# ZZWaang/polyphonic-chord-texture-disentanglement

Measured on AMD Instinct MI355X. Metric: 2-bar piano-roll samples/sec (train step), higher is better.
Workload: dtype bf16; 1 GPU; configs[1]: 1xMI355X batch=512/GPU, bf16 MFMA GRU/Linear, z_dim=256+256, teacher-forced decoder (tfr=1), fwd+bwd+clip+Adam; per_gpu_batch=512, global_batch=512, parallelism=dp1

## Files before the change

include/ptvae_hip.h:

```cpp
#ifndef PTVAE_HIP_H
#define PTVAE_HIP_H

#ifdef __cplusplus
extern "C" {
#endif

#define PTV_PREC_F32 0
#define PTV_PREC_BF16 1

#define PTV_A_BF16 1
#define PTV_B_BF16 2
#define PTV_C_BF16 4
#define PTV_GRU_GATES_BF16 1
#define PTV_GRU_GI_BF16 2
#define PTV_GRU_GI2_BF16 4
#define PTV_GRU_DG_BF16 8
#define PTV_GRU_W_BF16 16
#define PTV_GRU_EXT_BF16 64
#define PTV_GRU_SKIP_CAST0 32

const char* ptv_arch(void);
int ptv_abi_version(void);
const char* ptv_header_hash(void);

int ptv_gemm(int prec, int transA, int transB, int M, int N, int K,
             const void* A, long lda, const void* B, long ldb,
             void* C, long ldc, const float* bias, float alpha,
             int accumulate, int act, int splitk, int dtypes, void* stream);
int ptv_gemm_mtop(int prec, int transA, int transB, int M, int N, int K, const void* A, long lda, const void* B, long ldb,
                  void* C, long ldc, const float* bias, float alpha, int accumulate, int act, int splitk, int dtypes,
                  const int* m_top, long m_unit, void* stream);
int ptv_gemm_mtop_seg(int prec, int transA, int transB, int M, int N, int K, const void* A, long lda, const void* B, long ldb,
                      void* C, long ldc, const float* bias, float alpha, int accumulate, int act, int splitk, int dtypes,
                      const int* m_top, long m_unit, const int* seg_n, long seg_unit, int seg_period, void* stream);
int ptv_gemm_priority(int p);

int ptv_gru_seq_fwd(int prec, int M, int H, int T,
                    const void* gi, long gi_step_stride, long gi_ld,
                    const void* gi2, long gi2_step_stride, long gi2_ld,
                    const void* w_hh, const float* b_hh,
                    float* hall, void* hall16, void* gates,
                    const int* lengths, int reverse, const int* gi_idx, int flags, void* stream);

int ptv_gru_step_fwd(int prec, int M, int H,
                     const float* hprev, long ld_hprev, const void* hprev16, void* hout16,
                     const void* gi, long gi_ld, const void* gi2, long gi2_ld,
                     const void* w_hh, const float* b_hh,
                     float* hout, long ld_hout,
                     void* gates, long gates_plane,
                     const int* lengths, int t, const int* gi_idx, int flags, void* stream);

int ptv_gru_seq_bwd(int prec, int M, int H, int T,
                    const float* hall, const void* gates, const void* w_hh,
                    const void* dh_ext, long ext_step_stride, long ext_ld,
                    const float* dh_last, long last_ld,
                    const float* lr_a, long lr_step_stride, long lr_lda, int lr_k, const float* lr_b,
                    void* dgi, void* dgh, float* dhz, float* dh0,
                    int reverse, int flags, void* stream);

int ptv_gru_persist_supported(int NC, int M, int H);
int ptv_gru_persist_cu_reserve(int cus);
int ptv_gru_persist_load_policy(int lp);
int ptv_gru_persist_fwd(int NC, int M, int H, int T,
                        const void* const* gi, const long* gi_step, const long* gi_ld,
                        const void* const* gi2, const long* gi2_step, const long* gi2_ld,
                        const void* const* w_hh16, const float* const* b_hh,
                        float* const* hall, void* const* hall16, void* const* gates,
                        const int* const* lengths, const int* reverse, void* const* xch, unsigned* sync, void* stream);
int ptv_gru_persist_bwd(int NC, int M, int H, int T,
                        const float* const* hall, const void* const* gates, const void* const* w_t16,
                        const void* const* dh_ext, const long* ext_step, const long* ext_ld, const int* ext_bf16,
                        const float* const* dh_last, const long* last_ld,
                        void* const* dgi, void* const* dgh, float* const* dh0,
                        const int* reverse, void* const* xch, unsigned* sync, void* stream);
int ptv_gru_persist_splitk_supported(int NC, int M, int H, int S);
long ptv_gru_persist_part_elems(int NC, int M, int H, int S);
int ptv_gru_persist_bwd_splitk(int S, int NC, int M, int H, int T,
                               const float* const* hall, const void* const* gates, const void* const* w_t16,
                               const void* const* dh_ext, const long* ext_step, const long* ext_ld, const int* ext_bf16,
                               const float* const* dh_last, const long* last_ld,
                               void* const* dgi, void* const* dgh, float* const* dh0,
                               const int* reverse, void* const* xch, float* const* part, unsigned* sync, void* stream);

int ptv_copy2d(float* dst, long ldd, const float* src, long lds, long rows, int cols, float alpha,
               int accumulate, void* stream);
int ptv_transpose01(float* dst, const float* src, int D0, int D1, int W, void* stream);
int ptv_sum_steps(float* out, const void* in, long n, int T, long stride, int accumulate, int in_bf16, void* stream);
int ptv_zero_skip(int enable);
int ptv_last_nonzero_unit(const float* x, long rows, int cols, long ld, long unit, int* top, void* stream);
int ptv_sum_steps_top(float* out, const void* in, long n, int T, long stride, int accumulate, int in_bf16, const int* t_top,
                      void* stream);
int ptv_sum_steps_seg(float* out, const void* in, long n, int T, long stride, int accumulate, int in_bf16, const int* t_top,
                      const int* seg_n, long row_elems, void* stream);
int ptv_colsum(float* out, const void* A, long lda, long rows, int N, const int* sel, int G, int a_bf16, void* stream);

int ptv_embed_fwd(const long* x, const float* W, const float* bias, float* emb, int* lengths, int B, int E, void* stream);
int ptv_multihot(const long* x, float* out, long ld, int B, void* stream);
int ptv_grid_lengths(const long* x, int* lengths, int B, void* stream);
int ptv_multihot_bf16(const long* x, void* out, long ld, int B, void* stream);
int ptv_embed_fwd_geom(const long* x, const float* W, const float* bias, float* emb, int* lengths, int B, int E,
                       int S, int N, int P, int D, int pad, void* stream);
int ptv_grid_lengths_geom(const long* x, int* lengths, int B, int S, int N, int D, int pad, void* stream);
int ptv_multihot_geom(const long* x, void* out, long ld, int B, int S, int N, int P, int D, int bf16, void* stream);
int ptv_embed_multihot_fwd(const unsigned char* mh, const float* W, const float* bias, float* emb, int* lengths,
                           int B, int E, int S, int N, int K, int pad_col, void* stream);
int ptv_multihot_bytes_rows(const unsigned char* mh, void* out, long ld, int B, int S, int N, int K, int bf16, void* stream);

int ptv_txt_conv_relu_pool_fwd(const float* pr_mat, const float* w, const float* bias, float* pooled, int B, int C, void* stream);
int ptv_txt_conv_relu_pool_bwd(const float* pr_mat, const float* w, const float* bias, const float* dpooled,
                               float* dw, float* dbias, int B, int C, void* stream);
int ptv_txt_conv_relu_pool_fwd_rows(const float* pr_mat, const float* w, const float* bias, float* feat, long ld, int B, int C,
                                    signed char* arg, void* stream);
int ptv_txt_conv_relu_pool_bwd_rows(const float* pr_mat, const float* w, const float* bias, const float* dfeat, long ld,
                                    float* dw, float* dbias, int B, int C, const signed char* arg, void* stream);

int ptv_philox_normal(float* out, long rows, int Z, unsigned long long seed, unsigned long long stream_id, long row_offset,
                      void* stream);
// ... 119 lines not shown

enum PtvCdfTensor {
  PTV_CDF_Z = 0,
  PTV_CDF_C_SM,
  PTV_CDF_W_ZHID, PTV_CDF_B_ZHID, PTV_CDF_W_ZIN, PTV_CDF_B_ZIN, PTV_CDF_INIT_INPUT,
  PTV_CDF_W_IH,
  PTV_CDF_B_IH, PTV_CDF_W_HH, PTV_CDF_B_HH, PTV_CDF_W_ROOT, PTV_CDF_B_ROOT, PTV_CDF_W_CHROMA, PTV_CDF_B_CHROMA, PTV_CDF_W_BASS, PTV_CDF_B_BASS,
  PTV_CDF_HALL,
  PTV_CDF_Z_IN,
  PTV_CDF_TOKS,
  PTV_CDF_GI,
  PTV_CDF_ZG,
  PTV_CDF_GATES,
  PTV_CDF_ROOT, PTV_CDF_CHROMA, PTV_CDF_BASS,
  PTV_CDF_COUNT
};
enum PtvCdfDim { PTV_CDF_D_B = 0, PTV_CDF_D_T, PTV_CDF_D_H, PTV_CDF_D_I, PTV_CDF_D_Z, PTV_CDF_D_ZI, PTV_CDF_D_PREC, PTV_CDF_D_GATES_BF16,
                 PTV_CDF_D_NROOT, PTV_CDF_D_NCHROMA, PTV_CDF_D_NBASS, PTV_CDF_D_COUNT };
int ptv_chord_decoder_fwd(const void* const* t, const long* d, void* stream);

enum PtvCdbTensor {
  PTV_CDB_Z = 0,
  PTV_CDB_W_ZHID, PTV_CDB_W_ZIN, PTV_CDB_W_IH, PTV_CDB_W_HH, PTV_CDB_W_ROOT, PTV_CDB_W_CHROMA, PTV_CDB_W_BASS,
  PTV_CDB_WT16_HH,
  PTV_CDB_HALL, PTV_CDB_GATES, PTV_CDB_TOKS, PTV_CDB_Z_IN,
  PTV_CDB_DROOT, PTV_CDB_DCHROMA, PTV_CDB_DBASS,
  PTV_CDB_DZ,
  PTV_CDB_G_INIT_INPUT, PTV_CDB_G_W_ZHID, PTV_CDB_G_B_ZHID, PTV_CDB_G_W_ZIN, PTV_CDB_G_B_ZIN, PTV_CDB_G_W_IH, PTV_CDB_G_B_IH, PTV_CDB_G_W_HH,
  PTV_CDB_G_B_HH, PTV_CDB_G_W_ROOT, PTV_CDB_G_B_ROOT, PTV_CDB_G_W_CHROMA, PTV_CDB_G_B_CHROMA, PTV_CDB_G_W_BASS, PTV_CDB_G_B_BASS,
  PTV_CDB_DHS,
  PTV_CDB_DGI, PTV_CDB_DGH,
  PTV_CDB_DHZ,
  PTV_CDB_DH0,
  PTV_CDB_DZG,
  PTV_CDB_DZ_IN,
  PTV_CDB_DTOK0,
  PTV_CDB_XCH, PTV_CDB_PART, PTV_CDB_SYNC,
  PTV_CDB_WAIT_EVENT, PTV_CDB_RECORD_EVENT,
  PTV_CDB_COUNT
};
enum PtvCdbDim { PTV_CDB_D_B = 0, PTV_CDB_D_T, PTV_CDB_D_H, PTV_CDB_D_I, PTV_CDB_D_Z, PTV_CDB_D_ZI, PTV_CDB_D_PREC, PTV_CDB_D_ACT_BF16,
                 PTV_CDB_D_NROOT, PTV_CDB_D_NCHROMA, PTV_CDB_D_NBASS, PTV_CDB_D_PERSIST, PTV_CDB_D_SPLITK, PTV_CDB_D_COUNT };
int ptv_chord_decoder_bwd(const void* const* tensors, const long* dims, void* stream);

enum PtvDtbTensor {
  PTV_DTB_Z = 0,
  PTV_DTB_TOK_OP,
  PTV_DTB_DP,
  PTV_DTB_DDUR,
  PTV_DTB_TOP_H,
  PTV_DTB_W_HH_D, PTV_DTB_B_HH_D, PTV_DTB_W_IH_D, PTV_DTB_W_OUT_D, PTV_DTB_SOS,
  PTV_DTB_PK_WDPT, PTV_DTB_PK_WCAT,
  PTV_DTB_PK_NOTES_WT,
  PTV_DTB_WT_IH_N, PTV_DTB_WT_T2N, PTV_DTB_WT_IH_T, PTV_DTB_WT_HH_T, PTV_DTB_WT_ZHID, PTV_DTB_WT_ZIN,
  PTV_DTB_NS, PTV_DTB_NS16, PTV_DTB_Z_IN, PTV_DTB_TOKS, PTV_DTB_GATES_T, PTV_DTB_HN16, PTV_DTB_GATES_N, PTV_DTB_PITCH, PTV_DTB_HD16,
  PTV_DTB_TAB0, PTV_DTB_TAB, PTV_DTB_IDX,
  PTV_DTB_DZ,
  PTV_DTB_DTOK,
  PTV_DTB_DTOKS,
  PTV_DTB_G_W_ZHID, PTV_DTB_G_B_ZHID, PTV_DTB_G_W_ZIN, PTV_DTB_G_B_ZIN, PTV_DTB_G_INIT_INPUT,
  PTV_DTB_G_W_IH_T, PTV_DTB_G_W_HH_T, PTV_DTB_G_B_IH_T, PTV_DTB_G_B_HH_T,
  PTV_DTB_G_W_T2N, PTV_DTB_G_B_T2N,
  PTV_DTB_G_W_IH_N, PTV_DTB_G_W_HH_N, PTV_DTB_G_B_IH_N, PTV_DTB_G_B_HH_N,
  PTV_DTB_G_W_P, PTV_DTB_G_B_P, PTV_DTB_G_W_DH, PTV_DTB_G_B_DH, PTV_DTB_G_W_OUT_D, PTV_DTB_G_B_OUT_D,
  PTV_DTB_G_W_IH_D, PTV_DTB_G_W_HH_D, PTV_DTB_G_B_IH_D, PTV_DTB_G_B_HH_D, PTV_DTB_G_SOS,
  PTV_DTB_DHD0,
  PTV_DTB_PART,
  PTV_DTB_S,
  PTV_DTB_TMP64,
  PTV_DTB_DNSUM,
  PTV_DTB_DY16,
  PTV_DTB_TMP200,
  PTV_DTB_CS200,
  PTV_DTB_DGI_N, PTV_DTB_DGH_N, PTV_DTB_DHN0, PTV_DTB_SCRATCH_N,
  PTV_DTB_TOP_STEP,
  PTV_DTB_DGC, PTV_DTB_DNS,
  PTV_DTB_DGI_T, PTV_DTB_DGH_T, PTV_DTB_DZHID, PTV_DTB_DZG, PTV_DTB_DZ_IN,
  PTV_DTB_XCH, PTV_DTB_PART_T, PTV_DTB_SYNC,
  PTV_DTB_WAIT_EVENT, PTV_DTB_RECORD_EVENT,
  PTV_DTB_SIDE_STREAM,
  PTV_DTB_FORK_EVENT0, PTV_DTB_FORK_EVENT1, PTV_DTB_FORK_EVENT2, PTV_DTB_FORK_EVENT3,
  PTV_DTB_PERM, PTV_DTB_ROW_LEN,
  PTV_DTB_NS16S,
  PTV_DTB_DNS_S,
  PTV_DTB_DTOK_S,
  PTV_DTB_SEG_N,
  PTV_DTB_COUNT
};
enum PtvDtbDim { PTV_DTB_D_B = 0, PTV_DTB_D_E, PTV_DTB_D_HE, PTV_DTB_D_HT, PTV_DTB_D_HN, PTV_DTB_D_HD, PTV_DTB_D_NP, PTV_DTB_D_ZS, PTV_DTB_D_ZI,
                 PTV_DTB_D_LDP, PTV_DTB_D_NBLK, PTV_DTB_D_SPLITK, PTV_DTB_D_COUNT };
int ptv_decoder_tf_bwd(const void* const* tensors, const long* dims, void* stream);

enum PtvBgbTensor {
  PTV_BGB_X = 0,
  PTV_BGB_DOUT,
  PTV_BGB_HALL0, PTV_BGB_H16_0, PTV_BGB_GATES0, PTV_BGB_WT_HH0, PTV_BGB_WT_IH0,
  PTV_BGB_HALL1, PTV_BGB_H16_1, PTV_BGB_GATES1, PTV_BGB_WT_HH1, PTV_BGB_WT_IH1,
  PTV_BGB_G_W_IH0, PTV_BGB_G_W_HH0, PTV_BGB_G_B_IH0, PTV_BGB_G_B_HH0, PTV_BGB_G_W_IH1, PTV_BGB_G_W_HH1, PTV_BGB_G_B_IH1, PTV_BGB_G_B_HH1,
  PTV_BGB_DX,
  PTV_BGB_DGI0, PTV_BGB_DGH0, PTV_BGB_DGI1, PTV_BGB_DGH1,
  PTV_BGB_XCH0, PTV_BGB_XCH1, PTV_BGB_PART0, PTV_BGB_PART1, PTV_BGB_SYNC,
  PTV_BGB_WAIT_EVENT, PTV_BGB_RECORD_EVENT, PTV_BGB_SIDE_STREAM, PTV_BGB_FORK_EVENT, PTV_BGB_JOIN_EVENT,
  PTV_BGB_COUNT
};
enum PtvBgbDim { PTV_BGB_D_M = 0, PTV_BGB_D_T, PTV_BGB_D_H, PTV_BGB_D_I, PTV_BGB_D_X_BF16, PTV_BGB_D_DX_ACC, PTV_BGB_D_SPLITK, PTV_BGB_D_COUNT };
int ptv_bigru_final_bwd(const void* const* tensors, const long* dims, void* stream);

enum PtvBgfTensor {
  PTV_BGF_X = 0,
  PTV_BGF_LENGTHS,
  PTV_BGF_W16_IH0, PTV_BGF_B_IH0, PTV_BGF_W16_HH0, PTV_BGF_B_HH0, PTV_BGF_W16_IH1, PTV_BGF_B_IH1, PTV_BGF_W16_HH1, PTV_BGF_B_HH1,
  PTV_BGF_OUT,
  PTV_BGF_GI0, PTV_BGF_HALL0, PTV_BGF_H16_0, PTV_BGF_GATES0, PTV_BGF_GI1, PTV_BGF_HALL1, PTV_BGF_H16_1, PTV_BGF_GATES1,
  PTV_BGF_XCH0, PTV_BGF_XCH1, PTV_BGF_SYNC, PTV_BGF_WAIT_EVENT, PTV_BGF_RECORD_EVENT,
  PTV_BGF_COUNT
};
enum PtvBgfDim { PTV_BGF_D_M = 0, PTV_BGF_D_T, PTV_BGF_D_H, PTV_BGF_D_I, PTV_BGF_D_X_BF16,
                 PTV_BGF_D_WIH_F32,
                 PTV_BGF_D_COUNT };
int ptv_bigru_final_fwd(const void* const* tensors, const long* dims, void* stream);

enum PtvBrfTensor {
  PTV_BRF_X = 0,
  PTV_BRF_LENGTHS, PTV_BRF_PERM,
  PTV_BRF_PK_WG_H0, PTV_BRF_PK_WG_T0, PTV_BRF_B_HH0, PTV_BRF_B_IH0, PTV_BRF_PK_WG_H1, PTV_BRF_PK_WG_T1, PTV_BRF_B_HH1, PTV_BRF_B_IH1,
  PTV_BRF_OUT,
  PTV_BRF_HALL0, PTV_BRF_H16_0, PTV_BRF_GATES0, PTV_BRF_HALL1, PTV_BRF_H16_1, PTV_BRF_GATES1,
  PTV_BRF_SIDE_STREAM, PTV_BRF_FORK_EVENT, PTV_BRF_JOIN_EVENT,
  PTV_BRF_COUNT
};
enum PtvBrfDim { PTV_BRF_D_M = 0, PTV_BRF_D_T, PTV_BRF_D_H, PTV_BRF_D_I, PTV_BRF_D_COUNT };
int ptv_bigru_rows_fwd(const void* const* tensors, const long* dims, void* stream);
enum PtvBrbTensor {
  PTV_BRB_X = 0, PTV_BRB_DOUT, PTV_BRB_LENGTHS, PTV_BRB_PERM,
  PTV_BRB_PK_WT0, PTV_BRB_HALL0, PTV_BRB_H16_0, PTV_BRB_GATES0, PTV_BRB_WT_IH0,
  PTV_BRB_PK_WT1, PTV_BRB_HALL1, PTV_BRB_H16_1, PTV_BRB_GATES1, PTV_BRB_WT_IH1,
  PTV_BRB_G_W_IH0, PTV_BRB_G_W_HH0, PTV_BRB_G_B_IH0, PTV_BRB_G_B_HH0, PTV_BRB_G_W_IH1, PTV_BRB_G_W_HH1, PTV_BRB_G_B_IH1, PTV_BRB_G_B_HH1,
  PTV_BRB_DX,
  PTV_BRB_DGI0, PTV_BRB_DGH0, PTV_BRB_SCRATCH0, PTV_BRB_TOP0, PTV_BRB_DGI1, PTV_BRB_DGH1, PTV_BRB_SCRATCH1, PTV_BRB_TOP1,
  PTV_BRB_SIDE_STREAM, PTV_BRB_FORK_EVENT, PTV_BRB_JOIN_EVENT,
  PTV_BRB_SEG,
  PTV_BRB_COUNT
};
enum PtvBrbDim { PTV_BRB_D_M = 0, PTV_BRB_D_T, PTV_BRB_D_H, PTV_BRB_D_I, PTV_BRB_D_DX_ACC, PTV_BRB_D_DOUT_LD, PTV_BRB_D_COUNT };
int ptv_bigru_rows_bwd(const void* const* tensors, const long* dims, void* stream);

enum PtvVlTensor {
  PTV_VL_X = 0, PTV_VL_C,
  PTV_VL_PITCH, PTV_VL_DUR,
  PTV_VL_MU_C, PTV_VL_SD_C, PTV_VL_MU_R, PTV_VL_SD_R,
  PTV_VL_ROOT, PTV_VL_CHROMA, PTV_VL_BASS,
  PTV_VL_PITCH_T, PTV_VL_DUR_T, PTV_VL_COUNTS, PTV_VL_ROOT_T, PTV_VL_CHROMA_T, PTV_VL_BASS_T,
  PTV_VL_SUMS,
  PTV_VL_OUT,
  PTV_VL_GOUT,
  PTV_VL_GS,
  PTV_VL_DPITCH, PTV_VL_DDUR, PTV_VL_DMU_C, PTV_VL_DSD_C, PTV_VL_DMU_R, PTV_VL_DSD_R, PTV_VL_DROOT, PTV_VL_DCHROMA, PTV_VL_DBASS,
  PTV_VL_COUNT
};
enum PtvVlDim { PTV_VL_D_B = 0, PTV_VL_D_Z, PTV_VL_D_NP, PTV_VL_D_LDP, PTV_VL_D_SM_P, PTV_VL_D_SM_C, PTV_VL_D_HAVE_TARGETS, PTV_VL_D_COUNT };
int ptv_vae_loss_fwd(const void* const* tensors, const long* dims, const double* scal, void* stream);
int ptv_vae_loss_bwd(const void* const* tensors, const long* dims, const double* scal, void* stream);

int ptv_note_token(const float* pitch, long ld_pitch, const int* dur_idx, long dur_stride, const float* W, const float* bias, int E,
                   float* pred, long ld_pred, long* xhat, long xhat_stride, int* plen, int n, int last,
                   const int* force_pitch, int M, void* stream);
int ptv_chord_token(const float* root, const float* chroma, const float* bass, unsigned* masks2, float* token, int B, void* stream);
int ptv_route_slices(const float* src, float* dstA, float* dstB, const int* mask, long slice_elems, int nslices, int accumulate, void* stream);
// ... 30 lines not shown
int ptv_free_resummarize(const void* const* w, const void* const* io, int B, int t, int train, void* stream);

enum PtvDffTensor {
  PTV_DFF_Z = 0,
  PTV_DFF_XS,
  PTV_DFF_TOK0_SRC,
  PTV_DFF_W_ZHID, PTV_DFF_B_ZHID, PTV_DFF_W_ZIN, PTV_DFF_B_ZIN, PTV_DFF_W_IH_T, PTV_DFF_B_IH_T, PTV_DFF_INIT_INPUT, PTV_DFF_B_HH_T,
  PTV_DFF_W_IH_T_OP,
  PTV_DFF_W_HH_T_OP,
  PTV_DFF_W_CAT, PTV_DFF_B_CAT,
  PTV_DFF_W_IH_N, PTV_DFF_B_IH_N, PTV_DFF_B_HH_N, PTV_DFF_W_DH, PTV_DFF_B_DH, PTV_DFF_W_HH_D, PTV_DFF_B_HH_D, PTV_DFF_TAB0, PTV_DFF_TAB,
  PTV_DFF_W_OUT_D, PTV_DFF_B_OUT_D, PTV_DFF_PK_NOTES_H, PTV_DFF_PK_NOTES_T,
  PTV_DFF_PK_E_H0, PTV_DFF_PK_E_T0, PTV_DFF_B_HH_E0, PTV_DFF_B_IH_E0, PTV_DFF_PK_E_H1, PTV_DFF_PK_E_T1, PTV_DFF_B_HH_E1, PTV_DFF_B_IH_E1,
  PTV_DFF_NS, PTV_DFF_NS16, PTV_DFF_Z_IN, PTV_DFF_ZG, PTV_DFF_TOKS, PTV_DFF_GATES_T,
  PTV_DFF_GI, PTV_DFF_H0GC,
  PTV_DFF_TOK, PTV_DFF_PRED, PTV_DFF_PITCH, PTV_DFF_HN, PTV_DFF_HN16, PTV_DFF_GATES_N, PTV_DFF_HD, PTV_DFF_HD16, PTV_DFF_GATES_D,
  PTV_DFF_IDX, PTV_DFF_PLEN, PTV_DFF_GC16, PTV_DFF_DUR_SCR, PTV_DFF_IDX_SCR,
  PTV_DFF_XH0, PTV_DFF_XH1, PTV_DFF_XH16_0, PTV_DFF_XH16_1, PTV_DFF_XG0, PTV_DFF_XG1,
  PTV_DFF_WAIT_EVENT, PTV_DFF_RECORD_EVENT,
  PTV_DFF_SAMPLE,
  PTV_DFF_COUNT
};
enum PtvDffDim {
  PTV_DFF_D_B = 0, PTV_DFF_D_ZS, PTV_DFF_D_ZI, PTV_DFF_D_HE, PTV_DFF_D_HT, PTV_DFF_D_HN, PTV_DFF_D_HD, PTV_DFF_D_E, PTV_DFF_D_NP,
  PTV_DFF_D_LDP,
  PTV_DFF_D_TRAIN, PTV_DFF_D_REPLAY, PTV_DFF_D_INFERENCE,
  PTV_DFF_D_LOOP_FLAGS,
  PTV_DFF_D_CLUSTER,
  PTV_DFF_D_RESUM_TRAIN,
  PTV_DFF_D_TOK0_LDS,
  PTV_DFF_D_W_IH_T_BF16, PTV_DFF_D_W_HH_T_BF16,
  PTV_DFF_D_COUNT
};
int ptv_decoder_free_fwd(const void* const* t, const long* d, const void* const* wl, const void* const* io, const void* const* wr,
                         const void* const* ior, const unsigned* note_mask, const unsigned char* time_coin, void* stream);

enum PtvDfbTensor {
  PTV_DFB_DTOK = 0,
  PTV_DFB_DTOKS,
  PTV_DFB_DEMB, PTV_DFB_DPRED,
  PTV_DFB_DXS, PTV_DFB_DXSP,
  PTV_DFB_MASK_TOK, PTV_DFB_MASK_TIME,
  PTV_DFB_DX_PRED,
  PTV_DFB_XHAT,
  PTV_DFB_MH,
  PTV_DFB_G_W_EMB, PTV_DFB_G_B_EMB,
  PTV_DFB_COUNT
};
enum PtvDfbDim { PTV_DFB_D_B = 0, PTV_DFB_D_E, PTV_DFB_D_HE, PTV_DFB_D_COUNT };
int ptv_decoder_free_bwd(const void* const* t_tf, const long* d_tf, const void* const* t_rows, const long* d_rows, const void* const* t,
                         const long* d, void* stream);

int ptv_notes_gru_persist_fwd(const void* wg_h, const void* wg_t, const float* b_hh, const void* gc, const float* emb,
                              const float* h0, void* HN16, void* gates, long R, int T, void* stream);
int ptv_notes_gru_persist_fwd_top(const void* wg_h, const void* wg_t, const float* b_hh, const void* gc, const float* emb,
                                  const float* h0, void* HN16, void* gates, long R, int T, const int* live_top, void* stream);
long ptv_notes_gru_persist_scratch_elems(long R);
int ptv_notes_gru_persist_bwd(const void* wt, const void* HN16, const void* gates, const void* ext, void* dgi, void* dgh,
                              float* dh0, void* scratch, long R, int T, int* top_step, void* stream);
int ptv_notes_gru_persist_bwd_top(const void* wt, const void* HN16, const void* gates, const void* ext, void* dgi, void* dgh,
                                  float* dh0, void* scratch, long R, int T, const int* bound, int* top_step, void* stream);
int ptv_notes_gru_persist_fwd_rows(const void* wg_h, const void* wg_t, const float* b_hh, const void* gc, const float* emb,
                                   const float* h0, void* HN16, void* gates, long R, int T, const int* live_top, const int* row_len,
                                   void* stream);
int ptv_notes_gru_persist_bwd_rows(const void* wt, const void* HN16, const void* gates, const void* ext, void* dgi, void* dgh,
                                   float* dh0, void* scratch, long R, int T, const int* bound, const int* row_len, int* top_step,
                                   void* stream);
int ptv_notes_bwd_variant(int eight_waves);

int ptv_row_gru_persist_fwd(int H, const void* w_hh, const void* w_x, const float* b_hh, const float* b_ih, const void* gc,
                            const float* x, long x_step, const int* lengths, float* HN, void* HN16, void* gates,
                            float* out, long out_ld, long R, int T, int reverse, void* stream);
long ptv_row_gru_persist_scratch_elems(int H, long R);
int ptv_row_gru_persist_bwd(int H, const void* wt, const void* HN, const void* gates, const void* ext,
                            const float* dh_last, long last_ld, const int* lengths, void* dgi, void* dgh, float* dh0,
                            void* scratch, long R, int T, int reverse, int* top_step, void* stream);
int ptv_row_gru_persist_fwd_perm(int H, const void* w_hh, const void* w_x, const float* b_hh, const float* b_ih, const void* gc,
                                 const float* x, long x_step, const int* lengths, const int* perm, float* HN, void* HN16,
                                 void* gates, float* out, long out_ld, long R, int T, int reverse, void* stream);
int ptv_row_gru_persist_bwd_perm(int H, const void* wt, const void* HN, const void* gates, const void* ext,
                                 const float* dh_last, long last_ld, const int* lengths, const int* perm, void* dgi, void* dgh,
                                 float* dh0, void* scratch, long R, int T, int reverse, int* top_step, void* stream);
int ptv_rows_by_length(const int* lengths, int* perm, long R, int max_len, void* stream);

int ptv_cast_bf16(const float* src, void* dst, long n, void* stream);
int ptv_transpose_cast_bf16(const float* src, void* dst, int rows, int cols, void* stream);
int ptv_transpose_cast_bf16_batched(const float* flat, void* flat_t, const long* desc, int nmat, long ntiles, void* stream);
int ptv_grad_sumsq(const float* g, long n, float* sumsq, void* stream);
int ptv_clip_adam_step(float* p, const float* g, float* m, float* v, long n, const float* sumsq, float gscale, float clip,
                       float lr, float beta1, float beta2, float eps, int step, void* stream);
int ptv_clip_adam_step_shadow(float* p, const float* g, float* m, float* v, long n, const float* sumsq, float gscale, float clip,
                              float lr, float beta1, float beta2, float eps, int step, void* p16, void* stream);
int ptv_gradnorm_clip_adam_step(float* p, const float* g, float* m, float* v, long n, float* sumsq, float gscale, float clip,
                                float lr, float beta1, float beta2, float eps, int step, void* p16, void* stream);

int ptv_ordered_reductions(int on);
int ptv_wgrad_mode(int ordered);
int ptv_wgrad_dma(int enable);
long ptv_ordered_fallbacks(int reset);

int ptv_step_params(const float* dev4);

int ptv_wgrad(int M, int N, int K, const void* A, long lda, const void* B, long ldb, float* C, long ldc, float alpha,
              int accumulate, int dtypes, int slabs, float* colsum_a, const int* k_top, long k_unit, int k_rev, void* stream);
int ptv_wgrad_cat(int M1, const void* A1, long lda1, int M2, const void* A2, long lda2, int N, int K, const void* B, long ldb,
                  float* C, long ldc, float alpha, int accumulate, int dtypes, int slabs, float* colsum_a, const int* k_top,
                  long k_unit, int k_rev, void* stream);
typedef struct ptv_wgrad_job {
  int M, N, K;
  const void* A; long lda;
  const void* B; long ldb;
  float* C; long ldc;
  float alpha;
  int accumulate, dtypes, slabs;
  float* colsum_a;
  const int* k_top; long k_unit; int k_rev;
  const int* seg_n; long seg_unit; int seg_period;
} ptv_wgrad_job;
int ptv_wgrad_batch(const ptv_wgrad_job* jobs, int njobs, void* stream);
int ptv_wgrad_seg_supported(long K, long seg_unit);
int ptv_rows_seg_counts(const int* row_len, long R, int steps, int* seg_n, void* stream);


#ifdef __cplusplus
}
#endif
#endif
```

polyphonic_chord_texture_disentanglement_amd/csrc/composite.hip:

```cpp
#include "common.hpp"
#include "../../include/ptvae_hip.h"

namespace {

inline const void* T_(const void* const* t, int i) { return t[i]; }
template <typename X> inline X* M_(const void* const* t, int i) { return reinterpret_cast<X*>(const_cast<void*>(t[i])); }

constexpr int A16 = 1, B16 = 2, C16 = 4, CBLK16 = 16;

struct WgradGroup {
  ptv_wgrad_job jobs[8]; int n = 0; int P; void* stream;
  WgradGroup(int prec, void* st) : P(prec), stream(st) {}
  int add(int M, int N, long K, const void* A, long lda, int a_bf16, const void* B, long ldb, int b_bf16, float* C, long ldc, float* csum,
          const int* k_top = nullptr, long k_unit = 0, int k_rev = 0, int accumulate = 1, const int* seg_n = nullptr, long seg_unit = 0,
          int seg_period = 0) {
    if (P == PTV_PREC_BF16 && K >= 512) {
      if (n == 8) PTV_TRY(flush());
      jobs[n++] = ptv_wgrad_job{M, N, (int)K, A, lda, B, ldb, C, ldc, 1.f, accumulate, (a_bf16 ? 1 : 0) | (b_bf16 ? 2 : 0), 0, csum, k_top, k_unit, k_rev,
                                seg_n, seg_n ? seg_unit : 0, seg_n ? seg_period : 0};
      return PTV_OK;
    }
    if (k_top) return PTV_ERR_ARG;
    PTV_TRY(ptv_gemm(P, 1, 1, M, N, (int)K, A, lda, B, ldb, C, ldc, nullptr, 1.f, accumulate, 0, 0, (a_bf16 ? A16 : 0) | (b_bf16 ? B16 : 0), stream));
    if (csum) PTV_TRY(ptv_colsum(csum, A, lda, K, M, nullptr, 1, a_bf16, stream));
// ... 128 lines not shown
                   0, 0, 0, stream));
  return PTV_OK;
}

extern "C" int ptv_chord_decoder_bwd(const void* const* t, const long* d, void* stream) {
  if (!t || !d) return PTV_ERR_ARG;
  const int B = (int)d[PTV_CDB_D_B], T = (int)d[PTV_CDB_D_T], H = (int)d[PTV_CDB_D_H], I = (int)d[PTV_CDB_D_I], Z = (int)d[PTV_CDB_D_Z],
            Zi = (int)d[PTV_CDB_D_ZI], P = (int)d[PTV_CDB_D_PREC], abf = d[PTV_CDB_D_ACT_BF16] ? 1 : 0, persist = (int)d[PTV_CDB_D_PERSIST],
            S = (int)d[PTV_CDB_D_SPLITK];
  if (B <= 0 || T <= 0 || H <= 0 || I <= 0 || Z <= 0 || Zi <= 0 || (P != PTV_PREC_F32 && P != PTV_PREC_BF16)) return PTV_ERR_ARG;
  for (int i = 0; i < PTV_CDB_COUNT; i++) {
    const bool optional = i == PTV_CDB_WT16_HH || i == PTV_CDB_DROOT || i == PTV_CDB_DCHROMA || i == PTV_CDB_DBASS || i == PTV_CDB_DHZ ||
                          i == PTV_CDB_XCH || i == PTV_CDB_PART || i == PTV_CDB_SYNC || i == PTV_CDB_WAIT_EVENT || i == PTV_CDB_RECORD_EVENT;
    if (!t[i] && !optional) return PTV_ERR_ARG;
  }
  if (persist && (!t[PTV_CDB_WT16_HH] || !t[PTV_CDB_XCH] || !t[PTV_CDB_SYNC] || !abf || (S && !t[PTV_CDB_PART]))) return PTV_ERR_ARG;
  if (!persist && !t[PTV_CDB_DHZ]) return PTV_ERR_ARG;
  hipStream_t s = (hipStream_t)stream;
  const long TB = (long)T * B, ld_ih = (long)I + Zi;
  const float* hall = (const float*)T_(t, PTV_CDB_HALL);
  const float* hs = hall + (long)B * H;
  float* dhs = M_<float>(t, PTV_CDB_DHS);
  const int heads[3][4] = {{PTV_CDB_DROOT, PTV_CDB_W_ROOT, PTV_CDB_G_W_ROOT, PTV_CDB_G_B_ROOT},
                           {PTV_CDB_DCHROMA, PTV_CDB_W_CHROMA, PTV_CDB_G_W_CHROMA, PTV_CDB_G_B_CHROMA},
                           {PTV_CDB_DBASS, PTV_CDB_W_BASS, PTV_CDB_G_W_BASS, PTV_CDB_G_B_BASS}};
  const int ncls[3] = {(int)d[PTV_CDB_D_NROOT], (int)d[PTV_CDB_D_NCHROMA], (int)d[PTV_CDB_D_NBASS]};
  bool have = false;
  WgradGroup wg(P, stream);
  for (int k = 0; k < 3; k++) {
    const void* dl = T_(t, heads[k][0]);
    if (!dl) continue;
    const int n = ncls[k];
    PTV_TRY(ptv_gemm(P, 0, 1, (int)TB, H, n, dl, n, T_(t, heads[k][1]), H, dhs, H, nullptr, 1.f, have ? 1 : 0, 0, 0, 0, stream));
    have = true;
    PTV_TRY(wg.add(n, H, TB, dl, n, 0, hs, H, 0, M_<float>(t, heads[k][2]), H, M_<float>(t, heads[k][3])));
  }
  PTV_TRY(wg.flush());
  if (!have && hipMemsetAsync(dhs, 0, sizeof(float) * TB * H, s) != hipSuccess) return PTV_ERR_LAUNCH;
  void* dgi = M_<void>(t, PTV_CDB_DGI); void* dgh = M_<void>(t, PTV_CDB_DGH);
  float* dh0 = M_<float>(t, PTV_CDB_DH0);
  if (persist) {
    const float* hall_[1] = {hall}; const void* gates_[1] = {T_(t, PTV_CDB_GATES)}; const void* wt_[1] = {T_(t, PTV_CDB_WT16_HH)};
    const void* ext_[1] = {dhs}; const long ext_step[1] = {(long)B * H}, ext_ld[1] = {(long)H}; const int ext_bf[1] = {0};
    const float* last_[1] = {nullptr}; const long last_ld[1] = {0};
    void* dgi_[1] = {dgi}; void* dgh_[1] = {dgh}; float* dh0_[1] = {dh0}; const int rev[1] = {0};
    void* xch_[1] = {M_<void>(t, PTV_CDB_XCH)}; float* part_[1] = {M_<float>(t, PTV_CDB_PART)};
    if (t[PTV_CDB_WAIT_EVENT] && hipStreamWaitEvent(s, (hipEvent_t)const_cast<void*>(t[PTV_CDB_WAIT_EVENT]), 0) != hipSuccess) return PTV_ERR_LAUNCH;
    if (S) PTV_TRY(ptv_gru_persist_bwd_splitk(S, 1, B, H, T, hall_, gates_, wt_, ext_, ext_step, ext_ld, ext_bf, last_, last_ld, dgi_, dgh_, dh0_, rev,
                                              xch_, part_, M_<unsigned>(t, PTV_CDB_SYNC), stream));
    else PTV_TRY(ptv_gru_persist_bwd(1, B, H, T, hall_, gates_, wt_, ext_, ext_step, ext_ld, ext_bf, last_, last_ld, dgi_, dgh_, dh0_, rev, xch_,
                                     M_<unsigned>(t, PTV_CDB_SYNC), stream));
    if (t[PTV_CDB_RECORD_EVENT] && hipEventRecord((hipEvent_t)const_cast<void*>(t[PTV_CDB_RECORD_EVENT]), s) != hipSuccess) return PTV_ERR_LAUNCH;
  } else {
    const void* w = t[PTV_CDB_WT16_HH] ? T_(t, PTV_CDB_WT16_HH) : T_(t, PTV_CDB_W_HH);
    const int flags = abf | (abf << 3) | ((t[PTV_CDB_WT16_HH] ? 1 : 0) << 4);
    PTV_TRY(ptv_gru_seq_bwd(P, B, H, T, hall, T_(t, PTV_CDB_GATES), w, dhs, (long)B * H, H, nullptr, 0, nullptr, 0, 0, 0, nullptr, dgi, dgh,
                            M_<float>(t, PTV_CDB_DHZ), dh0, 0, flags, stream));
  }
  const int A = abf ? A16 : 0;
  float* dzg = M_<float>(t, PTV_CDB_DZG);
  PTV_TRY(ptv_sum_steps_top(dzg, dgi, (long)B * 3 * H, T, (long)B * 3 * H, 0, abf, nullptr, stream));
  float* g_ih = M_<float>(t, PTV_CDB_G_W_IH);
  const float* w_ih = (const float*)T_(t, PTV_CDB_W_IH);
  float* dz_in = M_<float>(t, PTV_CDB_DZ_IN); float* dtok0 = M_<float>(t, PTV_CDB_DTOK0);
  PTV_TRY(ptv_gemm(P, 0, 1, B, Zi, 3 * H, dzg, 3L * H, w_ih + I, ld_ih, dz_in, Zi, nullptr, 1.f, 0, 0, 0, 0, stream));
  PTV_TRY(ptv_gemm(P, 0, 1, B, I, 3 * H, dgi, 3L * H, w_ih, ld_ih, dtok0, I, nullptr, 1.f, 0, 0, 0, A, stream));
  float* dz = M_<float>(t, PTV_CDB_DZ);
  PTV_TRY(ptv_gemm(P, 0, 1, B, Z, H, dh0, H, T_(t, PTV_CDB_W_ZHID), Z, dz, Z, nullptr, 1.f, 0, 0, 0, 0, stream));
  PTV_TRY(ptv_gemm(P, 0, 1, B, Z, Zi, dz_in, Zi, T_(t, PTV_CDB_W_ZIN), Z, dz, Z, nullptr, 1.f, 1, 0, 0, 0, stream));
  PTV_TRY(wg.add(3 * H, H, TB, dgh, 3L * H, abf, hall, H, 0, M_<float>(t, PTV_CDB_G_W_HH), H, M_<float>(t, PTV_CDB_G_B_HH)));
  PTV_TRY(wg.add(3 * H, Zi, B, dzg, 3L * H, 0, T_(t, PTV_CDB_Z_IN), Zi, 0, g_ih + I, ld_ih, M_<float>(t, PTV_CDB_G_B_IH)));
  PTV_TRY(wg.add(3 * H, I, TB, dgi, 3L * H, abf, T_(t, PTV_CDB_TOKS), I, 0, g_ih, ld_ih, nullptr));
  PTV_TRY(wg.add(H, Z, B, dh0, H, 0, T_(t, PTV_CDB_Z), Z, 0, M_<float>(t, PTV_CDB_G_W_ZHID), Z, M_<float>(t, PTV_CDB_G_B_ZHID)));
  PTV_TRY(wg.add(Zi, Z, B, dz_in, Zi, 0, T_(t, PTV_CDB_Z), Z, 0, M_<float>(t, PTV_CDB_G_W_ZIN), Z, M_<float>(t, PTV_CDB_G_B_ZIN)));
  PTV_TRY(wg.flush());
  PTV_TRY(ptv_colsum(M_<float>(t, PTV_CDB_G_INIT_INPUT), dtok0, I, B, I, nullptr, 1, 0, stream));
  return PTV_OK;
}

extern "C" int ptv_decoder_tf_bwd(const void* const* t, const long* d, void* stream) {
  if (!t || !d) return PTV_ERR_ARG;
  for (int i = 0; i < PTV_DTB_COUNT; i++)
    if (!t[i] && i != PTV_DTB_TOP_H && i != PTV_DTB_PART_T && i != PTV_DTB_WAIT_EVENT && i != PTV_DTB_RECORD_EVENT && i != PTV_DTB_PERM &&
        i != PTV_DTB_ROW_LEN && i != PTV_DTB_NS16S && i != PTV_DTB_DNS_S && i != PTV_DTB_DTOK_S && i != PTV_DTB_SEG_N)
      return PTV_ERR_ARG;
  const bool sorted = t[PTV_DTB_PERM] != nullptr;
  if (sorted != (t[PTV_DTB_ROW_LEN] != nullptr) || sorted != (t[PTV_DTB_NS16S] != nullptr) || sorted != (t[PTV_DTB_DNS_S] != nullptr) ||
      sorted != (t[PTV_DTB_DTOK_S] != nullptr) || (sorted && !t[PTV_DTB_TOP_H]))
    return PTV_ERR_ARG;
  const int* perm = (const int*)T_(t, PTV_DTB_PERM);
  const int* row_len = (const int*)T_(t, PTV_DTB_ROW_LEN);

  const int B = (int)d[PTV_DTB_D_B], E = (int)d[PTV_DTB_D_E], He = (int)d[PTV_DTB_D_HE], Ht = (int)d[PTV_DTB_D_HT], Hn = (int)d[PTV_DTB_D_HN],
            Hd = (int)d[PTV_DTB_D_HD], NP = (int)d[PTV_DTB_D_NP], Zs = (int)d[PTV_DTB_D_ZS], Zi = (int)d[PTV_DTB_D_ZI], nblk = (int)d[PTV_DTB_D_NBLK],
            S = (int)d[PTV_DTB_D_SPLITK];
  const long ldp = d[PTV_DTB_D_LDP];
  if (B <= 0 || E != 128 || Hn != 512 || Hd != 64 || NP != 130 || ldp < NP || nblk <= 0 || (S && !t[PTV_DTB_PART_T])) return PTV_ERR_UNSUPPORTED;
  const int R = 32 * B;
  const int* seg_n = t[PTV_DTB_PERM] ? (const int*)T_(t, PTV_DTB_SEG_N) : nullptr;
  if (seg_n && !ptv_wgrad_seg_supported(15L * R, R)) return PTV_ERR_ARG;
  const long M = 15L * R;
  const int P = PTV_PREC_BF16;
  hipStream_t s = (hipStream_t)stream, side = (hipStream_t)const_cast<void*>(t[PTV_DTB_SIDE_STREAM]);
  void* sside = (void*)side;
  const int psz = ptv_dur_gru_bwd_part_size();
  const int* top_h = (const int*)T_(t, PTV_DTB_TOP_H);
  const long top_unit = top_h ? R : 0;
  auto fork = [&](int k) -> int {
    hipEvent_t e = (hipEvent_t)const_cast<void*>(t[PTV_DTB_FORK_EVENT0 + k]);
    if (hipEventRecord(e, s) != hipSuccess || hipStreamWaitEvent(side, e, 0) != hipSuccess) return PTV_ERR_LAUNCH;
    return PTV_OK;
  };
  float* G_ = nullptr; (void)G_;
#define GB(i) M_<float>(t, i)

  float* ddur = GB(PTV_DTB_DDUR); float* dHD0 = GB(PTV_DTB_DHD0); float* part = GB(PTV_DTB_PART);
  const void* HD16 = T_(t, PTV_DTB_HD16);
  ptv_gemm_priority(1);
  PTV_TRY(ptv_dur_gru_bwd(Hd, M, nullptr, M * Hd, 4 * M * Hd, HD16, M * Hd, 1, ddur, 10, (const float*)T_(t, PTV_DTB_W_HH_D),
                          (const float*)T_(t, PTV_DTB_W_OUT_D), (const int*)T_(t, PTV_DTB_IDX), M, dHD0, part, nblk,
                          (const float*)T_(t, PTV_DTB_B_HH_D), (const float*)T_(t, PTV_DTB_TAB0), (const float*)T_(t, PTV_DTB_TAB), stream));
  PTV_TRY(fork(0));
  ptv_gemm_priority(0);
  PTV_TRY(ptv_dur_out_wgrad(ddur, 10, HD16, M * Hd, GB(PTV_DTB_G_W_OUT_D), M, Hd, sside));
  PTV_TRY(ptv_colsum(GB(PTV_DTB_TMP64), ddur, 64, M * 10 / 64, 64, nullptr, 1, 0, sside));
  PTV_TRY(ptv_colsum(GB(PTV_DTB_G_B_OUT_D), GB(PTV_DTB_TMP64), 2, 32, 2, nullptr, 1, 0, sside));
  PTV_TRY(ptv_colsum(GB(PTV_DTB_S), part, psz, nblk, psz, nullptr, 1, 0, sside));
  PTV_TRY(ptv_dur_bwd_finalize(GB(PTV_DTB_S), GB(PTV_DTB_G_W_HH_D), GB(PTV_DTB_G_B_HH_D), GB(PTV_DTB_G_B_IH_D), GB(PTV_DTB_G_W_IH_D), GB(PTV_DTB_G_SOS),
                               (const float*)T_(t, PTV_DTB_W_IH_D), (const float*)T_(t, PTV_DTB_SOS), 5, sside));

  float* dP = GB(PTV_DTB_DP);
  void* dNSUM = M_<void>(t, PTV_DTB_DNSUM); void* dY16 = M_<void>(t, PTV_DTB_DY16);
  ptv_gemm_priority(1);
  PTV_TRY(ptv_heads_bwd_rows(dP, ldp, dHD0, T_(t, PTV_DTB_PK_WDPT), T_(t, PTV_DTB_PK_WCAT), dNSUM, top_h ? 3 : 1, dY16, top_h, top_unit, row_len, M,
                             stream));
  PTV_TRY(fork(1));
  ptv_gemm_priority(0);
  {
    const __bf16* HN16 = (const __bf16*)T_(t, PTV_DTB_HN16);
    const __bf16* nsum = HN16 + (long)R * Hn;
    float* tmp = GB(PTV_DTB_TMP200); float* cs = GB(PTV_DTB_CS200);
    WgradGroup wg(P, sside);
    PTV_TRY(wg.add(200, Hn, M, dY16, 200, 1, nsum, Hn, 1, tmp, Hn, cs, top_h, top_unit, 0, 0, seg_n, R, 15));
    PTV_TRY(wg.add(Hd, NP, M, dHD0, Hd, 0, T_(t, PTV_DTB_PITCH), ldp, 0, GB(PTV_DTB_G_W_DH) + Hn, (long)Hn + NP, nullptr, top_h, top_unit, 0, 1, seg_n, R, 15));
    PTV_TRY(wg.flush());
    PTV_TRY(ptv_copy2d(GB(PTV_DTB_G_W_P), Hn, tmp, Hn, NP, Hn, 1.f, 1, sside));
    PTV_TRY(ptv_copy2d(GB(PTV_DTB_G_B_P), NP, cs, NP, 1, NP, 1.f, 1, sside));
    PTV_TRY(ptv_copy2d(GB(PTV_DTB_G_W_DH), (long)Hn + NP, tmp + 136L * Hn, Hn, Hd, Hn, 1.f, 1, sside));
    PTV_TRY(ptv_copy2d(GB(PTV_DTB_G_B_DH), Hd, cs + 136, Hd, 1, Hd, 1.f, 1, sside));
  }

  void* dgi_n = M_<void>(t, PTV_DTB_DGI_N); void* dgh_n = M_<void>(t, PTV_DTB_DGH_N);
  float* dHN0 = GB(PTV_DTB_DHN0); int* top_step = M_<int>(t, PTV_DTB_TOP_STEP);
  float* dGC = GB(PTV_DTB_DGC);
  float* dNS_out = GB(PTV_DTB_DNS); float* dtok_out = GB(PTV_DTB_DTOK);
  float* dNS = sorted ? GB(PTV_DTB_DNS_S) : dNS_out;
  float* dtok = sorted ? GB(PTV_DTB_DTOK_S) : dtok_out;
  const __bf16* wt_ih_n = (const __bf16*)T_(t, PTV_DTB_WT_IH_N);
  ptv_gemm_priority(1);
  PTV_TRY(ptv_notes_gru_persist_bwd_rows(T_(t, PTV_DTB_PK_NOTES_WT), T_(t, PTV_DTB_HN16), T_(t, PTV_DTB_GATES_N), dNSUM, dgi_n, dgh_n, dHN0,
                                         M_<void>(t, PTV_DTB_SCRATCH_N), R, 15 | (seg_n ? 0x10000 : 0), top_h, row_len, top_step, stream));
  PTV_TRY(ptv_sum_steps_seg(dGC, dgi_n, (long)R * 3 * Hn, 15, (long)R * 3 * Hn, 0, 1, top_step, seg_n, 3L * Hn, stream));
  if (hipMemsetAsync(dtok_out + 15L * R * E, 0, sizeof(float) * R * E, s) != hipSuccess) return PTV_ERR_LAUNCH;
  PTV_TRY(ptv_gemm_mtop_seg(P, 0, 0, (int)M, E, 3 * Hn, dgi_n, 3L * Hn, wt_ih_n + (long)Ht * 3 * Hn, 3L * Hn, dtok, E, nullptr, 1.f, 0, 0, 0, A16 | B16,
                            top_step, R, seg_n, R, 15, stream));
  PTV_TRY(ptv_gemm(P, 0, 0, R, Ht, 3 * Hn, dGC, 3L * Hn, wt_ih_n, 3L * Hn, dNS, Ht, nullptr, 1.f, 0, 0, 0, B16, stream));
  PTV_TRY(ptv_gemm(P, 0, 0, R, Ht, Hn, dHN0, Hn, T_(t, PTV_DTB_WT_T2N), Hn, dNS, Ht, nullptr, 1.f, 1, 0, 0, B16, stream));
  if (sorted) {
    PTV_TRY(ptv_scatter_rows(dNS_out, dNS, perm, R, Ht, 0, 0, 1, stream));
    PTV_TRY(ptv_scatter_rows_seg(dtok_out, dtok, perm, R, E, (long)R * E, (long)R * E, 15, seg_n, stream));
  }
  PTV_TRY(fork(2));
  ptv_gemm_priority(0);
  {
    const __bf16* HN16 = (const __bf16*)T_(t, PTV_DTB_HN16);
    const __bf16* NSf = sorted ? (const __bf16*)T_(t, PTV_DTB_NS16S) : (const __bf16*)T_(t, PTV_DTB_NS16) + (long)B * Ht;
    float* gw = GB(PTV_DTB_G_W_HH_N); float* gb = GB(PTV_DTB_G_B_HH_N); float* gih = GB(PTV_DTB_G_W_IH_N);
    WgradGroup wg(P, sside);
    PTV_TRY(wg.add(2 * Hn, Hn, M, dgi_n, 3L * Hn, 1, HN16, Hn, 1, gw, Hn, gb, top_step, R, 0, 1, seg_n, R, 15));
    PTV_TRY(wg.add(Hn, Hn, M, dgh_n, Hn, 1, HN16, Hn, 1, gw + 2L * Hn * Hn, Hn, gb + 2 * Hn, top_step, R, 0, 1, seg_n, R, 15));
    PTV_TRY(wg.add(3 * Hn, Ht, R, dGC, 3L * Hn, 0, NSf, Ht, 1, gih, (long)Ht + E, GB(PTV_DTB_G_B_IH_N)));
    PTV_TRY(wg.add(3 * Hn, E, M, dgi_n, 3L * Hn, 1, T_(t, PTV_DTB_TOK_OP), E, 0, gih + Ht, (long)Ht + E, nullptr, top_step, R, 0, 1, seg_n, R, 15));
    PTV_TRY(wg.add(Hn, Ht, R, dHN0, Hn, 0, NSf, Ht, 1, GB(PTV_DTB_G_W_T2N), Ht, GB(PTV_DTB_G_B_T2N)));
    PTV_TRY(wg.flush());
  }

  void* dgi_t = M_<void>(t, PTV_DTB_DGI_T); void* dgh_t = M_<void>(t, PTV_DTB_DGH_T);
  float* dzhid = GB(PTV_DTB_DZHID); float* dZG = GB(PTV_DTB_DZG); float* dz_in = GB(PTV_DTB_DZ_IN); float* dTOKS = GB(PTV_DTB_DTOKS);
  float* dz = GB(PTV_DTB_DZ);
  const __bf16* wt_ih_t = (const __bf16*)T_(t, PTV_DTB_WT_IH_T);
  ptv_gemm_priority(1);
  {
    const float* hall_[1] = {(const float*)T_(t, PTV_DTB_NS)}; const void* gates_[1] = {T_(t, PTV_DTB_GATES_T)};
    const void* wt_[1] = {T_(t, PTV_DTB_WT_HH_T)};
    const void* ext_[1] = {dNS_out}; const long ext_step[1] = {(long)B * Ht}, ext_ld[1] = {(long)Ht}; const int ext_bf[1] = {0};
    const float* last_[1] = {nullptr}; const long last_ld[1] = {0};
    void* dgi_[1] = {dgi_t}; void* dgh_[1] = {dgh_t}; float* dh0_[1] = {dzhid}; const int rev[1] = {0};
    void* xch_[1] = {M_<void>(t, PTV_DTB_XCH)}; float* part_[1] = {M_<float>(t, PTV_DTB_PART_T)};
    if (t[PTV_DTB_WAIT_EVENT] && hipStreamWaitEvent(s, (hipEvent_t)const_cast<void*>(t[PTV_DTB_WAIT_EVENT]), 0) != hipSuccess) return PTV_ERR_LAUNCH;
    if (S) PTV_TRY(ptv_gru_persist_bwd_splitk(S, 1, B, Ht, 32, hall_, gates_, wt_, ext_, ext_step, ext_ld, ext_bf, last_, last_ld, dgi_, dgh_, dh0_,
                                              rev, xch_, part_, M_<unsigned>(t, PTV_DTB_SYNC), stream));
    else PTV_TRY(ptv_gru_persist_bwd(1, B, Ht, 32, hall_, gates_, wt_, ext_, ext_step, ext_ld, ext_bf, last_, last_ld, dgi_, dgh_, dh0_, rev, xch_,
                                     M_<unsigned>(t, PTV_DTB_SYNC), stream));
    if (t[PTV_DTB_RECORD_EVENT] && hipEventRecord((hipEvent_t)const_cast<void*>(t[PTV_DTB_RECORD_EVENT]), s) != hipSuccess) return PTV_ERR_LAUNCH;
  }
  PTV_TRY(ptv_sum_steps_top(dZG, dgi_t, (long)B * 3 * Ht, 32, (long)B * 3 * Ht, 0, 1, nullptr, stream));
  PTV_TRY(ptv_gemm(P, 0, 0, B, Zi, 3 * Ht, dZG, 3L * Ht, wt_ih_t + 2L * He * 3 * Ht, 3L * Ht, dz_in, Zi, nullptr, 1.f, 0, 0, 0, B16, stream));
  if (hipMemsetAsync(dTOKS + 32L * B * 2 * He, 0, sizeof(float) * B * 2 * He, s) != hipSuccess) return PTV_ERR_LAUNCH;
  PTV_TRY(ptv_gemm(P, 0, 0, R, 2 * He, 3 * Ht, dgi_t, 3L * Ht, wt_ih_t, 3L * Ht, dTOKS, 2L * He, nullptr, 1.f, 0, 0, 0, A16 | B16, stream));
  PTV_TRY(ptv_gemm(P, 0, 0, B, Zs, Ht, dzhid, Ht, T_(t, PTV_DTB_WT_ZHID), Ht, dz, Zs, nullptr, 1.f, 0, 0, 0, B16, stream));
  PTV_TRY(ptv_gemm(P, 0, 0, B, Zs, Zi, dz_in, Zi, T_(t, PTV_DTB_WT_ZIN), Zi, dz, Zs, nullptr, 1.f, 1, 0, 0, B16, stream));
  PTV_TRY(fork(3));
  ptv_gemm_priority(0);
  {
    const __bf16* NS16 = (const __bf16*)T_(t, PTV_DTB_NS16);
    float* g_ih = GB(PTV_DTB_G_W_IH_T); float* gb_ih = GB(PTV_DTB_G_B_IH_T); float* gb_hh = GB(PTV_DTB_G_B_HH_T);
    const long ld_t = 2L * He + Zi;
    WgradGroup wg(P, sside);
    PTV_TRY(wg.add(3 * Ht, Ht, R, dgh_t, 3L * Ht, 1, NS16, Ht, 1, GB(PTV_DTB_G_W_HH_T), Ht, gb_hh));
    PTV_TRY(wg.add(3 * Ht, Zi, B, dZG, 3L * Ht, 0, T_(t, PTV_DTB_Z_IN), Zi, 0, g_ih + 2 * He, ld_t, gb_ih));
    PTV_TRY(wg.add(3 * Ht, 2 * He, R, dgi_t, 3L * Ht, 1, T_(t, PTV_DTB_TOKS), 2L * He, 0, g_ih, ld_t, nullptr));
    PTV_TRY(wg.add(Ht, Zs, B, dzhid, Ht, 0, T_(t, PTV_DTB_Z), Zs, 0, GB(PTV_DTB_G_W_ZHID), Zs, GB(PTV_DTB_G_B_ZHID)));
    PTV_TRY(wg.add(Zi, Zs, B, dz_in, Zi, 0, T_(t, PTV_DTB_Z), Zs, 0, GB(PTV_DTB_G_W_ZIN), Zs, GB(PTV_DTB_G_B_ZIN)));
    PTV_TRY(wg.flush());
    PTV_TRY(ptv_colsum(GB(PTV_DTB_G_INIT_INPUT), dTOKS, 2L * He, B, 2 * He, nullptr, 1, 0, sside));
  }
  ptv_gemm_priority(1);
#undef GB
  return PTV_OK;
}

extern "C" int ptv_bigru_final_bwd(const void* const* t, const long* d, void* stream) {
  if (!t || !d) return PTV_ERR_ARG;
  const int M = (int)d[PTV_BGB_D_M], T = (int)d[PTV_BGB_D_T], H = (int)d[PTV_BGB_D_H], I = (int)d[PTV_BGB_D_I], xbf = d[PTV_BGB_D_X_BF16] ? 1 : 0,
            dx_acc = d[PTV_BGB_D_DX_ACC] ? 1 : 0, S = (int)d[PTV_BGB_D_SPLITK];
  if (M <= 0 || T < 2 || H <= 0 || I <= 0) return PTV_ERR_ARG;
  const bool want_dx = t[PTV_BGB_DX] != nullptr;
  for (int i = 0; i < PTV_BGB_COUNT; i++) {
    const bool optional = i == PTV_BGB_WT_IH0 || i == PTV_BGB_WT_IH1 || i == PTV_BGB_DX || i == PTV_BGB_PART0 || i == PTV_BGB_PART1 ||
                          i == PTV_BGB_WAIT_EVENT || i == PTV_BGB_RECORD_EVENT;
    if (!t[i] && !optional) return PTV_ERR_ARG;
  }
  if ((want_dx && (!t[PTV_BGB_WT_IH0] || !t[PTV_BGB_WT_IH1])) || (S && (!t[PTV_BGB_PART0] || !t[PTV_BGB_PART1]))) return PTV_ERR_ARG;
  const int P = PTV_PREC_BF16;
  hipStream_t s = (hipStream_t)stream, side = (hipStream_t)const_cast<void*>(t[PTV_BGB_SIDE_STREAM]);
  void* sside = (void*)side;
  const long TM = (long)T * M;
  const float* dout = (const float*)T_(t, PTV_BGB_DOUT);
  void* dgi[2] = {M_<void>(t, PTV_BGB_DGI0), M_<void>(t, PTV_BGB_DGI1)};
  void* dgh[2] = {M_<void>(t, PTV_BGB_DGH0), M_<void>(t, PTV_BGB_DGH1)};
  ptv_gemm_priority(1);
  {
    const float* hall_[2] = {(const float*)T_(t, PTV_BGB_HALL0), (const float*)T_(t, PTV_BGB_HALL1)};
    const void* gates_[2] = {T_(t, PTV_BGB_GATES0), T_(t, PTV_BGB_GATES1)};
    const void* wt_[2] = {T_(t, PTV_BGB_WT_HH0), T_(t, PTV_BGB_WT_HH1)};
    const void* ext_[2] = {nullptr, nullptr}; const long ext_step[2] = {0, 0}, ext_ld[2] = {0, 0}; const int ext_bf[2] = {0, 0};
    const float* last_[2] = {dout, dout + H}; const long last_ld[2] = {2L * H, 2L * H};
    float* dh0_[2] = {nullptr, nullptr}; const int rev[2] = {0, 1};
    void* xch_[2] = {M_<void>(t, PTV_BGB_XCH0), M_<void>(t, PTV_BGB_XCH1)};
    float* part_[2] = {M_<float>(t, PTV_BGB_PART0), M_<float>(t, PTV_BGB_PART1)};
    if (t[PTV_BGB_WAIT_EVENT] && hipStreamWaitEvent(s, (hipEvent_t)const_cast<void*>(t[PTV_BGB_WAIT_EVENT]), 0) != hipSuccess) return PTV_ERR_LAUNCH;
    if (S) PTV_TRY(ptv_gru_persist_bwd_splitk(S, 2, M, H, T, hall_, gates_, wt_, ext_, ext_step, ext_ld, ext_bf, last_, last_ld, dgi, dgh, dh0_, rev,
                                              xch_, part_, M_<unsigned>(t, PTV_BGB_SYNC), stream));
    else PTV_TRY(ptv_gru_persist_bwd(2, M, H, T, hall_, gates_, wt_, ext_, ext_step, ext_ld, ext_bf, last_, last_ld, dgi, dgh, dh0_, rev, xch_,
                                     M_<unsigned>(t, PTV_BGB_SYNC), stream));
    if (t[PTV_BGB_RECORD_EVENT] && hipEventRecord((hipEvent_t)const_cast<void*>(t[PTV_BGB_RECORD_EVENT]), s) != hipSuccess) return PTV_ERR_LAUNCH;
  }
  const void* x = T_(t, PTV_BGB_X);
  auto products = [&](int dir, void* st) -> int {
    const int o = dir ? 4 : 0;
    WgradGroup wg(P, st);
    PTV_TRY(wg.add(3 * H, I, TM, dgi[dir], 3L * H, 1, x, I, xbf, M_<float>(t, PTV_BGB_G_W_IH0 + o), I, M_<float>(t, PTV_BGB_G_B_IH0 + o)));
    PTV_TRY(wg.add(3 * H, H, TM, dgh[dir], 3L * H, 1, T_(t, dir ? PTV_BGB_H16_1 : PTV_BGB_H16_0), H, 1, M_<float>(t, PTV_BGB_G_W_HH0 + o), H,
                   M_<float>(t, PTV_BGB_G_B_HH0 + o), nullptr, 0, dir ? T : 0));
    return wg.flush();
  };
  hipEvent_t ef = (hipEvent_t)const_cast<void*>(t[PTV_BGB_FORK_EVENT]), ej = (hipEvent_t)const_cast<void*>(t[PTV_BGB_JOIN_EVENT]);
  if (hipEventRecord(ef, s) != hipSuccess || hipStreamWaitEvent(side, ef, 0) != hipSuccess) return PTV_ERR_LAUNCH;
// ... 332 lines not shown
```

polyphonic_chord_texture_disentanglement_amd/csrc/gemm.hip:

```cpp
#include <stdlib.h>
#include <mutex>
#include <type_traits>
#include "common.hpp"
#include "gemm_core.hpp"
#include "../../include/ptvae_hip.h"

namespace ptv {

struct EpiPlain {
  struct Params {
    void* C; long ldc;
    const float* bias;
    float alpha;
    int accumulate;
    int act;
    int atomic;
    int c_bf16;
    int c_blocked;
    int c_rows;
    long split_stride;
  };
  static __device__ __forceinline__ long coff(const Params& p, int m, int n) {
    return p.c_blocked ? (((long)(n >> p.c_blocked) * p.c_rows + m) << p.c_blocked) + (n & ((1 << p.c_blocked) - 1)) : (long)m * p.ldc + n;
  }
  static __device__ __forceinline__ bool dead_is_noop(const Params& p) { return (p.accumulate || p.atomic) && p.act == 0 && p.bias == nullptr; }
  template <int FM, int FN, int NG> struct Pre {};
  template <int FM, int FN, int NG>
  static __device__ __forceinline__ void prefetch(const Params&, Pre<FM, FN, NG>&, int, int, int, int) {}
  template <int FN> static constexpr bool staged() { return FN == 2 || FN == 4; }
  template <int FM, int FN, int NG> static constexpr int lds_bytes() { return staged<FN>() ? 4 * RowStage<1, (staged<FN>() ? FN * 16 : 64)>::WAVE_BYTES : 0; }
  template <int FM, int FN, int NG>
  static __device__ __forceinline__ void apply(const Params& p_in, f32x4 (&acc)[FM][NG * FN], const Pre<FM, FN, NG>&,
                                               int m0, int n0, int M, int N, int split, char* lds) {
    Params q = p_in;
    if (q.split_stride) q.C = reinterpret_cast<float*>(q.C) + (long)split * q.split_stride;
    const Params& p = q;
    const bool bf = p.c_bf16 != 0;
    const bool vec = (p.c_blocked || (p.ldc & 3) == 0) && ((reinterpret_cast<uintptr_t>(p.C) & (bf ? 7 : 15)) == 0);
    const bool use_bias = p.bias != nullptr && split == 0;
    if constexpr (staged<FN>()) {
      using RS = RowStage<1, FN * 16>;
      float* st = RS::base(lds);
      const int u = RS::unit();
      const bool bias_ok = !use_bias || (reinterpret_cast<uintptr_t>(p.bias) & 15) == 0;
      if (vec && bias_ok && p.act == 0 && m0 + 16 * FM <= M && n0 + 16 * FN <= N && !(bf && p.atomic)) {
        const int mode = p.atomic ? 3 : (p.accumulate ? (bf ? 4 : 2) : (bf ? 1 : 0));
        float4 b4 = make_float4(0.f, 0.f, 0.f, 0.f);
        if (use_bias) b4 = *reinterpret_cast<const float4*>(p.bias + n0 + u);
        if (mode == 0) fast_rows<FM, FN, 0>(p, acc, st, m0, n0 + u, b4);
        else if (mode == 1) fast_rows<FM, FN, 1>(p, acc, st, m0, n0 + u, b4);
        else if (mode == 2) fast_rows<FM, FN, 2>(p, acc, st, m0, n0 + u, b4);
        else if (mode == 4) fast_rows<FM, FN, 4>(p, acc, st, m0, n0 + u, b4);
        else fast_rows<FM, FN, 3>(p, acc, st, m0, n0 + u, b4);
        return;
      }
#pragma unroll
      for (int i = 0; i < FM; i++) {
        RS::put(st, acc[i]);
#pragma unroll
        for (int c = 0; c < RS::PASSES; c++) {
          const int row = RS::row(c), m = m0 + i * 16 + row, n = n0 + u;
          if (m < M && n < N) cell(p, m, n, N, RS::get(st, row, u), bf, vec, use_bias);
        }
        __builtin_amdgcn_wave_barrier();
      }
    } else {
      const int lane = threadIdx.x & 63;
#pragma unroll
      for (int i = 0; i < FM; i++)
#pragma unroll
        for (int j = 0; j < FN; j++) {
          const int m = m0 + i * 16 + (lane & 15), n = n0 + j * 16 + (lane >> 4) * 4;
          if (m < M && n < N) cell(p, m, n, N, acc[i][j], bf, vec, use_bias);
        }
    }
  }
  template <int FM, int FN, int MODE>
  static __device__ __forceinline__ void fast_rows(const Params& p, f32x4 (&acc)[FM][FN], float* st, int m0, int n, const float4& b4) {
    using RS = RowStage<1, FN * 16>;
    const int u = RS::unit();
#pragma unroll
    for (int i = 0; i < FM; i++) {
      RS::put(st, acc[i]);
#pragma unroll
      for (int c = 0; c < RS::PASSES; c++) {
        const int row = RS::row(c);
        const f32x4 a = RS::get(st, row, u);
        const long off = coff(p, m0 + i * 16 + row, n);
        float v0 = p.alpha * a[0] + b4.x, v1 = p.alpha * a[1] + b4.y, v2 = p.alpha * a[2] + b4.z, v3 = p.alpha * a[3] + b4.w;
        if constexpr (MODE == 1 || MODE == 4) {
          if constexpr (MODE == 4) {
            const bf16x4 q = *reinterpret_cast<const bf16x4*>(reinterpret_cast<const __bf16*>(p.C) + off);
            v0 += (float)q[0]; v1 += (float)q[1]; v2 += (float)q[2]; v3 += (float)q[3];
          }
          bf16x4 o; o[0] = (__bf16)v0; o[1] = (__bf16)v1; o[2] = (__bf16)v2; o[3] = (__bf16)v3;
          *reinterpret_cast<bf16x4*>(reinterpret_cast<__bf16*>(p.C) + off) = o;
        } else if constexpr (MODE == 3) {
          float* cp = reinterpret_cast<float*>(p.C) + off;
          atomicAdd(cp, v0); atomicAdd(cp + 1, v1); atomicAdd(cp + 2, v2); atomicAdd(cp + 3, v3);
        } else {
          float4* cp = reinterpret_cast<float4*>(reinterpret_cast<float*>(p.C) + off);
          if constexpr (MODE == 2) { const float4 q = *cp; v0 += q.x; v1 += q.y; v2 += q.z; v3 += q.w; }
          *cp = make_float4(v0, v1, v2, v3);
        }
      }
      __builtin_amdgcn_wave_barrier();
    }
  }
  static __device__ __forceinline__ void cell(const Params& p, int m, int n, int N, const f32x4& a, bool bf, bool vec, bool use_bias) {
    float v[4];
#pragma unroll
    for (int e = 0; e < 4; e++) {
      v[e] = p.alpha * a[e];
      if (use_bias && n + e < N) v[e] += p.bias[n + e];
      if (p.act == 1) v[e] = expf(v[e]);
    }
    const long off = coff(p, m, n);
    if (p.atomic) {
      float* c = reinterpret_cast<float*>(p.C) + off;
#pragma unroll
      for (int e = 0; e < 4; e++) if (n + e < N) atomicAdd(c + e, v[e]);
    } else if (vec && n + 3 < N) {
      if (p.accumulate) { const float4 q = ld4f(p.C, off, bf); v[0] += q.x; v[1] += q.y; v[2] += q.z; v[3] += q.w; }
      st4f(p.C, off, bf, v[0], v[1], v[2], v[3]);
    } else {
#pragma unroll
      for (int e = 0; e < 4; e++) if (n + e < N) st1f(p.C, off + e, bf, p.accumulate ? ld1f(p.C, off + e, bf) + v[e] : v[e]);
    }
  }
};

#ifndef PTV_PF_TN
#define PTV_PF_TN 3
#endif
#ifndef PTV_PF_NT
#define PTV_PF_NT 2
#endif
#define PLAIN_PF_BIG(KA, KB, SA, SB) ((SA) && (SB) ? ((KA) ? PTV_PF_TN : PTV_PF_NT) : 1)

template <class CT, int BM, int BN, int WGM, int WGN, bool KA, bool KB, bool SA, bool SB>
__global__ __launch_bounds__(NTHREADS, 2) void gemm_plain_kernel(GemmArgs g, EpiPlain::Params ep) {
  if (g.prio) __builtin_amdgcn_s_setprio(3);
  gemm_body<CT, BM, BN, WGM, WGN, 1, KA, KB, EpiPlain, SA, SB, (BM * BN <= 64 * 64 ? 2 : PLAIN_PF_BIG(KA, KB, SA, SB))>(g, ep);
}

__global__ void splitk_reduce_kernel(float* __restrict__ C, long ldc, const float* __restrict__ ws, int M, int N, int splits, int accumulate) {
  const long total = (long)M * N;
  for (long i = (long)blockIdx.x * blockDim.x + threadIdx.x; i < total; i += (long)gridDim.x * blockDim.x) {
    float sum = 0.f;
    for (int z = 0; z < splits; z++) sum += ws[(long)z * total + i];
    float* cp = C + (i / N) * ldc + (i % N);
    *cp = (accumulate ? *cp : 0.f) + sum;
  }
}

__global__ void fill_rows_kernel(float* C, long ldc, int M, int N, float v) {
  long i = (long)blockIdx.x * blockDim.x + threadIdx.x;
  long total = (long)M * N;
  for (; i < total; i += (long)gridDim.x * blockDim.x) C[(i / N) * ldc + (i % N)] = v;
}

template <class CT, int BM, int BN, bool KA, bool KB, bool SA, bool SB>
static void launch_plain(const GemmArgs& g, const EpiPlain::Params& ep, int splits, hipStream_t s) {
  dim3 grid(cdiv(g.N, BN), cdiv(g.M, BM), splits);
  hipLaunchKernelGGL((gemm_plain_kernel<CT, BM, BN, 2, 2, KA, KB, SA, SB>), grid, dim3(NTHREADS), 0, s, g, ep);
}

int g_splitk_ordered = [] { const char* e = getenv("PTV_WGRAD_ORDERED"); return (e && e[0] == '0') ? 0 : 1; }();

static float* splitk_workspace(hipStream_t s, size_t bytes) {
  struct Buf { float* p; size_t bytes; };
  static Buf pool[64]; static hipStream_t keys[64]; static int n = 0; static std::mutex mu;
  std::lock_guard<std::mutex> lock(mu);
  int i = 0;
  for (; i < n; i++) if (keys[i] == s) break;
  if (i == n) { if (n == 64) return nullptr; keys[n++] = s; pool[i] = Buf{nullptr, 0}; }
  Buf& b = pool[i];
  if (b.bytes < bytes) {
    hipStreamCaptureStatus st = hipStreamCaptureStatusNone;
    if (hipStreamIsCapturing(s, &st) == hipSuccess && st != hipStreamCaptureStatusNone) return nullptr;
    const size_t want = bytes + bytes / 4;
    if (hipMalloc(reinterpret_cast<void**>(&b.p), want) != hipSuccess) { b = Buf{nullptr, 0}; return nullptr; }
    b.bytes = want;
  }
  return b.p;
}

template <class CT, bool SA, bool SB>
static int gemm_dispatch(int transA, int transB, GemmArgs g, EpiPlain::Params ep, int splitk, hipStream_t s) {
  const long blocks_big = (long)cdiv(g.M, 128) * cdiv(g.N, 128);
  const bool deepk = transA && g.K >= 4096;
  const bool big = blocks_big >= 192 || (deepk && g.M >= 256 && g.N >= 256);
  const int bm = big ? 128 : 64;
  long blocks = (long)cdiv(g.M, bm) * cdiv(g.N, bm);
  int splits = 1;
  if (splitk > 0) splits = splitk;
  else if (splitk == 0 && blocks < 256 && g.K >= 8 * CT::BK && ep.act == 0 && !ep.c_bf16) {
    const long target = deepk ? (big ? 640 : 1536) : 512;
    splits = (int)((target + blocks - 1) / blocks);
    int maxs = g.K / (4 * CT::BK);
    if (splits > maxs) splits = maxs;
    if (splits > 192) splits = 192;
    if (splits < 1) splits = 1;
  }
  if (g.K == 0) splits = 1;
  int kper = g.K;
  if (splits > 1) {
    if (splits >= 8) splits = (splits + 7) / 8 * 8;
    kper = cdiv(cdiv(g.K, splits), CT::BK) * CT::BK;
    const int s2 = cdiv(g.K, kper);
    if (s2 != splits && (s2 & 7) != 0 && s2 >= 8) {
      splits = s2 / 8 * 8;
      kper = cdiv(cdiv(g.K, splits), CT::BK) * CT::BK;
      splits = cdiv(g.K, kper);
    } else splits = s2;
  }
  g.k_per_split = kper;
  float* ws = nullptr;
  const EpiPlain::Params ep_user = ep;
  if (splits > 1 && g_splitk_ordered) {
    ws = splitk_workspace(s, (size_t)splits * g.M * g.N * sizeof(float));
    if (!ws) g_ord_fallbacks++;
  }
  if (ws) {
    ep.C = ws; ep.ldc = g.N; ep.accumulate = 0; ep.atomic = 0; ep.split_stride = (long)g.M * g.N;
  } else if (splits > 1) {
    ep.atomic = 1;
    if (!ep.accumulate) {
      long total = (long)g.M * g.N;
      int nb = (int)((total + 255) / 256); if (nb > 2048) nb = 2048;
      hipLaunchKernelGGL(fill_rows_kernel, dim3(nb), dim3(256), 0, s, reinterpret_cast<float*>(ep.C), ep.ldc, g.M, g.N, 0.f);
    }
  }
#define PTV_LAUNCH(KA, KB)                                              \
  do {                                                                  \
    if (big) launch_plain<CT, 128, 128, KA, KB, SA, SB>(g, ep, splits, s);      \
    else launch_plain<CT, 64, 64, KA, KB, SA, SB>(g, ep, splits, s);            \
  } while (0)
  if (!transA && !transB) PTV_LAUNCH(false, false);
  else if (!transA && transB) PTV_LAUNCH(false, true);
  else if (transA && transB) PTV_LAUNCH(true, true);
  else PTV_LAUNCH(true, false);
#undef PTV_LAUNCH
  if (ws) {
    const long total = (long)g.M * g.N;
    int nb = (int)((total + 255) / 256); if (nb > 2048) nb = 2048;
    hipLaunchKernelGGL(splitk_reduce_kernel, dim3(nb), dim3(256), 0, s, reinterpret_cast<float*>(ep_user.C), ep_user.ldc, ws, g.M, g.N, splits, ep_user.accumulate);
  }
  return PTV_OK;
}

}

namespace ptv { int g_gemm_prio = 0; }
extern "C" int ptv_gemm_priority(int p) { ptv::g_gemm_prio = p ? 1 : 0; return PTV_OK; }

extern "C" int ptv_gemm_mtop(int prec, int transA, int transB, int M, int N, int K,
                             const void* A, long lda, const void* B, long ldb,
                             void* C, long ldc, const float* bias, float alpha,
                             int accumulate, int act, int splitk, int dtypes, const int* m_top, long m_unit, void* stream) {
  return ptv_gemm_mtop_seg(prec, transA, transB, M, N, K, A, lda, B, ldb, C, ldc, bias, alpha, accumulate, act, splitk, dtypes, m_top, m_unit, nullptr, 0, 0,
                           stream);
}

extern "C" int ptv_gemm_mtop_seg(int prec, int transA, int transB, int M, int N, int K,
                                 const void* A, long lda, const void* B, long ldb,
                                 void* C, long ldc, const float* bias, float alpha,
                                 int accumulate, int act, int splitk, int dtypes, const int* m_top, long m_unit,
                                 const int* seg_n, long seg_unit, int seg_period, void* stream) {
  if (M < 0 || N < 0 || K < 0 || !A || !B || !C) return PTV_ERR_ARG;
  if (M == 0 || N == 0) return PTV_OK;
  const bool sa = dtypes & 1, sb = dtypes & 2, sc = dtypes & 4;
  if ((sa || sb) && prec != PTV_PREC_BF16) return PTV_ERR_ARG;
  if (sc && splitk > 1) return PTV_ERR_ARG;
  if (act != 0 && splitk > 1) return PTV_ERR_ARG;
  if ((dtypes & 8) && (dtypes & 16)) return PTV_ERR_ARG;
  if ((dtypes & 8) && ((N & 31) || splitk > 1)) return PTV_ERR_ARG;
  if ((dtypes & 16) && ((N & 15) || splitk > 1)) return PTV_ERR_ARG;
  if ((dtypes & 24) && splitk == 0) splitk = 1;
  if (prec == PTV_PREC_BF16 && transA && transB && !sc && !(dtypes & 24) && !bias && act == 0 && K >= 512 && splitk <= 0)
    return ptv_wgrad(M, N, K, A, lda, B, ldb, reinterpret_cast<float*>(C), ldc, alpha, accumulate, dtypes & 3, 0, nullptr, nullptr, 0, 0, stream);
  if (m_top && (transA || m_unit <= 0)) return PTV_ERR_ARG;
  if (seg_n && (transA || seg_unit <= 0 || (seg_unit & 127) || seg_period <= 0)) return PTV_ERR_ARG;
  ptv::GemmArgs g{A, lda, B, ldb, M, N, K, K, 0, m_top, m_unit, ptv::g_gemm_prio, seg_n, (int)seg_unit, seg_period};
  ptv::EpiPlain::Params ep{C, ldc, bias, alpha, accumulate, act, 0, sc ? 1 : 0, (dtypes & 8) ? 5 : ((dtypes & 16) ? 4 : 0), M, 0};
  hipStream_t s = (hipStream_t)stream;
  int rc;
  if (prec != PTV_PREC_BF16) rc = ptv::gemm_dispatch<ptv::F32, false, false>(transA, transB, g, ep, splitk, s);
  else if (sa && sb) rc = ptv::gemm_dispatch<ptv::BF16, true, true>(transA, transB, g, ep, splitk, s);
  else if (sa) rc = ptv::gemm_dispatch<ptv::BF16, true, false>(transA, transB, g, ep, splitk, s);
  else if (sb) rc = ptv::gemm_dispatch<ptv::BF16, false, true>(transA, transB, g, ep, splitk, s);
  else rc = ptv::gemm_dispatch<ptv::BF16, false, false>(transA, transB, g, ep, splitk, s);
  if (rc != PTV_OK) return rc;
  PTV_CHECK_LAUNCH();
  return PTV_OK;
}

extern "C" int ptv_gemm(int prec, int transA, int transB, int M, int N, int K,
                        const void* A, long lda, const void* B, long ldb,
                        void* C, long ldc, const float* bias, float alpha,
                        int accumulate, int act, int splitk, int dtypes, void* stream) {
  return ptv_gemm_mtop(prec, transA, transB, M, N, K, A, lda, B, ldb, C, ldc, bias, alpha, accumulate, act, splitk, dtypes, nullptr, 0, stream);
}
```

polyphonic_chord_texture_disentanglement_amd/csrc/notes_persist.hip:

```cpp
#include "common.hpp"
#include "gemm_core.hpp"
#include "prof.hpp"
#include "../../include/ptvae_hip.h"

namespace ptv {

extern int g_gemm_prio;

__device__ __forceinline__ long gate_off(long row, int u, long R) { return ((long)(u >> 5) * R + row) * 32 + (u & 31); }
__device__ __forceinline__ long ext_off(int s, long row, int u, long R, int T) { return ((long)(u >> 5) * ((long)T * R) + (long)s * R + row) * 32 + (u & 31); }

constexpr int NE = 128, NRP = 64;
constexpr int NT16LD = NE + 16;

__device__ __forceinline__ float nsig(float x) { return __builtin_amdgcn_rcpf(1.0f + __expf(-x)); }
__device__ __forceinline__ float ntanh(float x) { return 1.0f - 2.0f * __builtin_amdgcn_rcpf(1.0f + __expf(2.0f * x)); }

__device__ __forceinline__ void pair_to_rows(const f32x4& f0, const f32x4& f1, float (&o)[8]) {
#pragma unroll
  for (int e = 0; e < 4; e++) { o[e] = f0[e]; o[4 + e] = f1[e]; }
}

typedef __attribute__((ext_vector_type(4))) float f4v;
__device__ __forceinline__ bf16x8 ldnt_bf16x8(const __bf16* p) { return __builtin_nontemporal_load(reinterpret_cast<const bf16x8*>(p)); }
// ... 516 lines not shown
          stnt_bf16x8(ph, dr); stnt_bf16x8(ph + H, dz); stnt_bf16x8(ph + 2 * H, dnr);
        } else {
          stnt_bf16x8(a.dgh + (long)s * RH + grow[i] * H + u, dnr);
        }
        __bf16* pi = a.dgi + (long)tt * R3H + gnat[i] * (3 * H) + u;
        stnt_bf16x8(pi, dr); stnt_bf16x8(pi + H, dz); stnt_bf16x8(pi + 2 * H, dn);
      }
    }
    __syncthreads();
  }
}

template <int H, bool EMB>
__global__ __launch_bounds__(256, H == 128 ? 2 : 1) void row_gru_bwd_kernel(RowGruBwdArgs a) {
  __builtin_amdgcn_s_setprio(3);
  extern __shared__ __attribute__((aligned(16))) char nsm[];
  row_gru_bwd_body<H, EMB>(a, blockIdx.x, nsm);
}

constexpr long ROW_GRU_MAX_R = 0x7fffffffL;
static inline bool aligned16(const void* p) { return (reinterpret_cast<unsigned long long>(p) & 15) == 0; }

template <int H, bool EMB>
static int launch_fwd(const RowGruFwdArgs& a, hipStream_t s) {
  const size_t lds = (size_t)(2 * NRP * (H + 16) + NRP * NT16LD) * sizeof(__bf16) + 16;
  static bool attr = false;
  if (!attr) {
    if (hipFuncSetAttribute(reinterpret_cast<const void*>(row_gru_fwd_kernel<H, EMB>), hipFuncAttributeMaxDynamicSharedMemorySize, (int)lds) != hipSuccess) return PTV_ERR_LAUNCH;
    attr = true;
  }
  hipLaunchKernelGGL((row_gru_fwd_kernel<H, EMB>), dim3((unsigned)((a.R + NRP - 1) / NRP)), dim3(256), lds, s, a);
  return PTV_OK;
}
template <int H, bool EMB>
static int launch_bwd(const RowGruBwdArgs& a, hipStream_t s) {
  const size_t lds = (size_t)NRP * H * sizeof(float);
  static bool attr = false;
  if (!attr) {
    if (hipFuncSetAttribute(reinterpret_cast<const void*>(row_gru_bwd_kernel<H, EMB>), hipFuncAttributeMaxDynamicSharedMemorySize, (int)lds) != hipSuccess) return PTV_ERR_LAUNCH;
    attr = true;
  }
  hipLaunchKernelGGL((row_gru_bwd_kernel<H, EMB>), dim3((unsigned)((a.R + NRP - 1) / NRP)), dim3(256), lds, s, a);
  return PTV_OK;
}

__global__ __launch_bounds__(1024) void rows_by_length_kernel(const int* __restrict__ lengths, int* __restrict__ perm, long R, int nb) {
  extern __shared__ int cnt[];
  int* wtot = cnt + nb * 1024;
  int* base = wtot + nb * 16;
  const int tid = threadIdx.x, lane = tid & 63, wave = tid >> 6;
  const long chunk = (R + 1023) / 1024, r0 = tid * chunk, r1 = min(R, r0 + chunk);
  for (int b = 0; b < nb; b++) cnt[b * 1024 + tid] = 0;
  for (long r = r0; r < r1; r++) cnt[min(max(lengths[r], 0), nb - 1) * 1024 + tid]++;
  for (int b = 0; b < nb; b++) {
    const int v = cnt[b * 1024 + tid];
    int incl = v;
#pragma unroll
    for (int d = 1; d < 64; d <<= 1) {
      const int o = __shfl_up(incl, d, 64);
      if (lane >= d) incl += o;
    }
    if (lane == 63) wtot[b * 16 + wave] = incl;
    cnt[b * 1024 + tid] = incl - v;
  }
  __syncthreads();
  if (tid < nb) {
    int run = 0;
    for (int w = 0; w < 16; w++) { const int t = wtot[tid * 16 + w]; wtot[tid * 16 + w] = run; run += t; }
    base[tid] = run;
  }
  __syncthreads();
  if (tid == 0) {
    int run = 0;
    for (int b = nb - 1; b >= 0; b--) { const int t = base[b]; base[b] = run; run += t; }
  }
  __syncthreads();
  for (long r = r0; r < r1; r++) {
    const int b = min(max(lengths[r], 0), nb - 1);
    const int pos = base[b] + wtot[b * 16 + wave] + cnt[b * 1024 + tid]++;
    perm[pos] = (int)r;
  }
}

}

using namespace ptv;

extern "C" int ptv_rows_by_length(const int* lengths, int* perm, long R, int max_len, void* stream) {
  if (!lengths || !perm || R <= 0 || R > 0x7fffffffL || max_len < 0) return PTV_ERR_ARG;
  const int nb = max_len + 1;
  const size_t lds = (size_t)(nb * 1024 + nb * 16 + nb) * sizeof(int);
  if (lds > 160 * 1024) return PTV_ERR_UNSUPPORTED;
  static bool attr = false;
  if (!attr) {
    if (hipFuncSetAttribute(reinterpret_cast<const void*>(rows_by_length_kernel), hipFuncAttributeMaxDynamicSharedMemorySize, 160 * 1024) != hipSuccess) return PTV_ERR_LAUNCH;
    attr = true;
  }
  hipLaunchKernelGGL(rows_by_length_kernel, dim3(1), dim3(1024), lds, (hipStream_t)stream, lengths, perm, R, nb);
  PTV_CHECK_LAUNCH();
  return PTV_OK;
}

extern "C" int ptv_notes_bwd8(const void* wt, const void* HN16, const void* gates, const void* ext, void* dgi, void* dgh, float* dh0, void* scratch,
                              long R, int T, const int* bound, const int* row_len, int* top_step, void* stream);
static int g_notes_bwd8 = 1;
extern "C" int ptv_notes_bwd_variant(int eight_waves) { g_notes_bwd8 = eight_waves ? 1 : 0; return PTV_OK; }

extern "C" int ptv_row_gru_persist_fwd_perm(int H, const void* w_hh, const void* w_x, const float* b_hh, const float* b_ih, const void* gc,
                                            const float* x, long x_step, const int* lengths, const int* perm, float* HN, void* HN16,
                                            void* gates, float* out, long out_ld, long R, int T, int reverse, void* stream);
extern "C" int ptv_row_gru_persist_fwd(int H, const void* w_hh, const void* w_x, const float* b_hh, const float* b_ih, const void* gc,
                                       const float* x, long x_step, const int* lengths, float* HN, void* HN16, void* gates,
                                       float* out, long out_ld, long R, int T, int reverse, void* stream) {
  return ptv_row_gru_persist_fwd_perm(H, w_hh, w_x, b_hh, b_ih, gc, x, x_step, lengths, nullptr, HN, HN16, gates, out, out_ld, R, T, reverse, stream);
}

extern "C" int ptv_row_gru_persist_fwd_perm(int H, const void* w_hh, const void* w_x, const float* b_hh, const float* b_ih, const void* gc,
                                            const float* x, long x_step, const int* lengths, const int* perm, float* HN, void* HN16,
                                            void* gates, float* out, long out_ld, long R, int T, int reverse, void* stream) {
  if (!w_hh || !w_x || !b_hh || !x || !HN || !HN16 || R <= 0 || T <= 0 || (T & 0xff) == 0 || (H != 512 && H != 128)) return PTV_ERR_ARG;
  if (out && (out_ld & 3)) return PTV_ERR_ARG;
  if ((x_step & 3) || !aligned16(x) || !aligned16(HN) || !aligned16(out)) return PTV_ERR_ARG;
  if (H == 128 && (T & ~0xff)) return PTV_ERR_ARG;
  if (R > ROW_GRU_MAX_R) return PTV_ERR_UNSUPPORTED;
  if (H == 512) {
    if (!gc || b_ih || lengths || perm || reverse || out || x_step != R * NE) return PTV_ERR_UNSUPPORTED;
    return ptv_notes_gru_persist_fwd(w_hh, w_x, b_hh, gc, x, HN, HN16, gates, R, T, stream);
  }
  RowGruFwdArgs a{(const bf16x8*)w_hh, (const bf16x8*)w_x, b_hh, b_ih, (const __bf16*)gc, x, x_step, lengths, HN, (__bf16*)HN16,
                  (__bf16*)gates, out, out_ld, (int)R, T & 0xff, reverse, 0, g_zero_skip, g_gemm_prio, perm};
  const int pi = prof::want(3, (int)R, H) ? prof::begin((hipStream_t)stream) : -1;
  if (gc || !b_ih) return PTV_ERR_UNSUPPORTED;
  PTV_TRY((launch_fwd<128, true>(a, (hipStream_t)stream)));
  if (pi >= 0) prof::end(pi, (hipStream_t)stream, 2.0 * R * 3.0 * H * (H + NE) * (T & 0xff));
  PTV_CHECK_LAUNCH();
  return PTV_OK;
}

extern "C" long ptv_row_gru_persist_scratch_elems(int H, long R) { return ((R + NRP - 1) / NRP) * 2 * ((3L * H / 8) * NRP * 8); }

extern "C" int ptv_row_gru_persist_bwd_perm(int H, const void* wt, const void* HN, const void* gates, const void* ext,
                                            const float* dh_last, long last_ld, const int* lengths, const int* perm, void* dgi, void* dgh,
                                            float* dh0, void* scratch, long R, int T, int reverse, int* top_step, void* stream);
static int row_gru_bwd_any(int H, const void* wt, const void* HN, const void* gates, const void* ext, const float* dh_last, long last_ld,
                           const int* lengths, const int* perm, void* dgi, void* dgh, float* dh0, void* scratch, long R, int T, int reverse,
                           const int* bound, const int* row_len, int* top_step, void* stream);
extern "C" int ptv_row_gru_persist_bwd(int H, const void* wt, const void* HN, const void* gates, const void* ext,
                                       const float* dh_last, long last_ld, const int* lengths, void* dgi, void* dgh, float* dh0,
                                       void* scratch, long R, int T, int reverse, int* top_step, void* stream) {
  return ptv_row_gru_persist_bwd_perm(H, wt, HN, gates, ext, dh_last, last_ld, lengths, nullptr, dgi, dgh, dh0, scratch, R, T, reverse, top_step, stream);
}

extern "C" int ptv_row_gru_persist_bwd_perm(int H, const void* wt, const void* HN, const void* gates, const void* ext,
                                            const float* dh_last, long last_ld, const int* lengths, const int* perm, void* dgi, void* dgh,
                                            float* dh0, void* scratch, long R, int T, int reverse, int* top_step, void* stream) {
  return row_gru_bwd_any(H, wt, HN, gates, ext, dh_last, last_ld, lengths, perm, dgi, dgh, dh0, scratch, R, T, reverse, nullptr, nullptr, top_step, stream);
}

static int row_gru_bwd_any(int H, const void* wt, const void* HN, const void* gates, const void* ext, const float* dh_last, long last_ld,
                           const int* lengths, const int* perm, void* dgi, void* dgh, float* dh0, void* scratch, long R, int T, int reverse,
                           const int* bound, const int* row_len, int* top_step, void* stream) {
  if (!wt || !HN || !gates || !dgi || !dgh || !scratch || R <= 0 || T <= 0 || (T & 0xff) == 0 || (H != 512 && H != 128)) return PTV_ERR_ARG;
  if (dh_last && (last_ld & 3)) return PTV_ERR_ARG;
  if (H == 128 && ((T & ~0xff) || !aligned16(HN))) return PTV_ERR_ARG;
  if (R > ROW_GRU_MAX_R) return PTV_ERR_UNSUPPORTED;
  T &= 0xff;
  if (H == 512 && (lengths || perm)) return PTV_ERR_UNSUPPORTED;
  if (perm && dh0) return PTV_ERR_UNSUPPORTED;
  RowGruBwdArgs a{(const bf16x8*)wt, H == 512 ? nullptr : (const float*)HN, H == 512 ? (const __bf16*)HN : nullptr, (const __bf16*)gates, (const __bf16*)ext, dh_last, last_ld, lengths, top_step, (__bf16*)dgi, (__bf16*)dgh, dh0,
                  (__bf16*)scratch, (int)R, T, reverse, g_zero_skip, perm, bound, row_len};
  const int pi = prof::want(4, (int)R, H) ? prof::begin((hipStream_t)stream) : -1;
  if (H == 512 && (!ext || dh_last || reverse)) return PTV_ERR_UNSUPPORTED;
  if (H == 128 && ext) return PTV_ERR_UNSUPPORTED;
  PTV_TRY(H == 512 ? (launch_bwd<512, false>(a, (hipStream_t)stream)) : (launch_bwd<128, true>(a, (hipStream_t)stream)));
  if (pi >= 0) prof::end(pi, (hipStream_t)stream, 2.0 * R * 3.0 * H * H * (T - 1 + (dh0 ? 1 : 0)));
  PTV_CHECK_LAUNCH();
  return PTV_OK;
}

extern "C" long ptv_notes_gru_persist_scratch_elems(long R) { return ptv_row_gru_persist_scratch_elems(512, R); }

// ... 17 lines not shown
```

polyphonic_chord_texture_disentanglement_amd/functional.py:

```python
import collections
import contextlib
import ctypes
import os
import time
import weakref

import torch

from . import _lib as _libmod
from ._lib import SlotTable, call, check, lib, prec_code, ptr, stream_ptr


_get_cur = getattr(torch._C, '_cuda_getCurrentStream', None)
_get_dev = getattr(torch._C, '_cuda_getDevice', None)
_set_stream = getattr(torch._C, '_cuda_setStream', None)


def cur_stream():
    if _get_cur is None or _get_dev is None:
        return torch.cuda.current_stream()
    sid, di, dt = _get_cur(_get_dev())
    return torch.cuda.Stream(stream_id=sid, device_index=di, device_type=dt)

F32 = torch.float32
# ... 949 lines not shown
        dx = dx_acc if dx_acc is not None else _empty(T * M, I, dev=dev)
    tens = {'X': xf, 'DOUT': dout, 'LENGTHS': state.lengths, 'PERM': state.perm, 'DX': dx, 'SEG': state.seg}
    for d_ in range(2):
        pk = notes_packs(w[4 * d_], w[4 * d_ + 1], 0)
        dgi, dgh, scratch, top = _bigru_bwd_buffers(state, T, M, H, dev)
        tens.update({'PK_WT%d' % d_: pk['wt'], 'HALL%d' % d_: state.hall[d_], 'H16_%d' % d_: state.h16[d_], 'GATES%d' % d_: state.gates[d_],
                     'WT_IH%d' % d_: wt_ih[d_], 'DGI%d' % d_: dgi, 'DGH%d' % d_: dgh, 'SCRATCH%d' % d_: scratch, 'TOP%d' % d_: top})
    evs = _fork_events('BRB')
    arr_ = _BRB.pointers(tens, dict(zip(_BIGRU_G, G)),
                         handles={'FORK_EVENT': evs[0].cuda_event, 'JOIN_EVENT': evs[1].cuda_event, 'SIDE_STREAM': side.s.cuda_stream})
    darr_ = _BRB.dims({'M': M, 'T': T, 'H': H, 'I': I, 'DX_ACC': dx_acc is not None, 'DOUT_LD': dout.stride(0)})
    sp_ = stream_ptr()
    rc = _defer_or_run('rows_bwd', (arr_, darr_, (tens, G, state, dout, xf)), lambda: lib().ptv_bigru_rows_bwd(arr_, darr_, sp_))
    _SIDE_DEPTH[1] = 1
    if rc == -3:
        raise RuntimeError('ptv_bigru_rows_bwd refused a configuration its Python-side checks accepted')
    check(rc, 'ptv_bigru_rows_bwd')
    _BRB.count()
    return G[0:4] + G[4:8], (dx.view(T, M, I) if need_dx else None)


def _bigru_fwd_composite(prec, xf, lengths, w, w16, out, T, M, I, H, dev):
    wih16 = [_W(w[0], prec), _W(w[4], prec)]
    if (torch.cuda.is_current_stream_capturing() or xf.dtype not in (F32, BF16) or xf.stride(1) != 1 or xf.stride(0) != I
            or wih16[0].dtype != wih16[1].dtype or not wih16[0].is_contiguous() or not wih16[1].is_contiguous()):
        return None
    dims = {'M': M, 'T': T, 'H': H, 'I': I, 'X_BF16': _bf(xf), 'WIH_F32': wih16[0].dtype == F32}
    dirs = []
    tens = {'X': xf, 'LENGTHS': lengths, 'OUT': out, 'SYNC': _persist_sync(2, dev)}
    for d_ in range(2):
        hall, gates, h16 = _bigru_fwd_buffers(T, M, H, dev, BF16, False)
        dirs.append((hall, gates, h16))
        tens.update({'W16_IH%d' % d_: wih16[d_], 'B_IH%d' % d_: w[4 * d_ + 2], 'W16_HH%d' % d_: w16[d_], 'B_HH%d' % d_: w[4 * d_ + 3],
                     'GI%d' % d_: _empty(T * M, 3 * H, dev=dev, dtype=BF16), 'HALL%d' % d_: hall, 'H16_%d' % d_: h16, 'GATES%d' % d_: gates,
                     'XCH%d' % d_: torch.empty((T + 1) * M * H, device=dev, dtype=BF16)})
    turn = _CompositeTurn(cur_stream())
    slots = _BGF.pointers(tens, handles=turn.handles)
    _chain_prio()
    rc = lib().ptv_bigru_final_fwd(slots, _BGF.dims(dims), stream_ptr())
    if rc == -3:
        return None
    check(rc, 'ptv_bigru_final_fwd')
    turn.taken()
    _BGF.count()
    return BiGruState('persist', dirs)


def _bigru_forward(prec, x3, lengths, w):
    T, M, I = x3.shape
    H = w[1].shape[1]
    dev = x3.device
    xf = x3.reshape(T * M, I)
    out = _empty(M, 2 * H, dev=dev)
    adt = _act_dtype(prec, H)
    w16 = [_W(w[1], prec), _W(w[5], prec)]
    branch = _bigru_branch(prec, x3, w16, adt, T, M, I, H)

    def gi_of(d):
        return gemm(xf, _W(w[4 * d], prec), bias=w[4 * d + 2], prec=prec, out_dtype=adt)

    if branch == 'persist':
        if BIGRU_BWD_COMPOSITE:
            state = _bigru_fwd_composite(prec, xf, lengths, w, w16, out, T, M, I, H, dev)
            if state is not None:
                return out, state
        chains, dirs = [], []
        for d in range(2):
            gi = gi_of(d)
            hall, gates, h16 = _bigru_fwd_buffers(T, M, H, dev, adt, True)
            chains.append(dict(gi=gi, gi_step=M * 3 * H, gi_ld=3 * H, w16=w16[d], b_hh=w[4 * d + 3], hall=hall, hall16=h16, gates=gates,
                               lengths=lengths, reverse=bool(d)))
            dirs.append((hall, gates, h16))
        gru_persist_fwd(M, H, T, chains)
        for d in range(2):
            copy2d(out[:, d * H:(d + 1) * H], dirs[d][0][T])
        return out, BiGruState('persist', dirs)

    zero_skip_sync()
    side = Side(BIGRU_SLOT)
    skip_by, perm, seg = None, None, None
    if branch == 'rows':
        skip_by = lengths if ZERO_SKIP else None
        if lengths is not None and ZERO_SKIP and SORT_ROWS and T <= 38:
            perm = torch.empty(M, device=dev, dtype=torch.int32)
            call('ptv_rows_by_length', ptr(lengths), ptr(perm), M, T, stream_ptr())
            if WGRAD_SEG and M % 128 == 0 and lib().ptv_wgrad_seg_supported(T * M, M):
                len_s = torch.empty(M, device=dev, dtype=torch.int32)
                call('ptv_gather_rows', ptr(len_s), ptr(lengths), ptr(perm), M, 1, 0, 0, 1, stream_ptr())
                seg = torch.empty(T, device=dev, dtype=torch.int32)
                call('ptv_rows_seg_counts', ptr(len_s), M, T, ptr(seg), stream_ptr())
        if BIGRU_BWD_COMPOSITE:
            state = _bigru_rows_fwd_composite(x3, lengths, skip_by, perm, seg, w, out, side, T, M, I, H, dev)
            if state is not None:
                return out, state

        def run(d):
            w_ih, w_hh, b_ih, b_hh = w[4 * d: 4 * d + 4]
            pk = notes_packs(w_ih, w_hh, 0)
            hall, gates, h16 = _bigru_fwd_buffers(T, M, H, dev, BF16, True)
            call('ptv_row_gru_persist_fwd_perm', H, ptr(pk['wg_h']), ptr(pk['wg_t']), ptr(b_hh), ptr(b_ih), None, ptr(x3), M * I,
                 ptr(lengths) if lengths is not None else None, ptr(perm), ptr(hall), ptr(h16), ptr(gates), out.data_ptr() + 4 * d * H,
                 2 * H, M, T, d, stream_ptr())
            return hall, gates, h16
    else:
        def run(d):
            gi = gi_of(d)
            hall, gates, h16 = _bigru_fwd_buffers(T, M, H, dev, adt, True)
            gru_fwd(prec, gi, M * 3 * H, 3 * H, w[4 * d + 1], w[4 * d + 3], hall, gates, lengths=lengths, reverse=bool(d), hall16=h16)
            copy2d(out[:, d * H:(d + 1) * H], hall[T])
            return hall, gates, h16
    rev = side(lambda: run(1), x3, out)
    fwd = run(0)
    side.join()
    return out, BiGruState(branch, [fwd, rev], skip_by, perm, seg)


BIGRU_BWD_COMPOSITE = os.environ.get('PTV_BWD_COMPOSITES', '1') != '0'


def _bigru_bwd_composite(prec, x3, xf, w, state, dout, need_dx, dx_acc, wts, side, T, M, I, H):
    dev = x3.device
    if (T * M < 512 or not OVERLAP or side.s == side.main or torch.cuda.is_current_stream_capturing() or xf.stride(1) != 1
            or xf.stride(0) != I or xf.dtype not in (F32, BF16) or dout.dtype != F32 or dout.stride(1) != 1 or dout.stride(0) != 2 * H):
        return None
    wt_ih = [_WT(w[0], prec), _WT(w[4], prec)] if need_dx else [None, None]
    if need_dx and (wt_ih[0] is None or wt_ih[1] is None):
        return None
    S = persist_splitk(2, M, H)
    dims = {'M': M, 'T': T, 'H': H, 'I': I, 'X_BF16': _bf(xf), 'DX_ACC': dx_acc is not None, 'SPLITK': S}
    G = [_gbuf(p_) for p_ in w]
    dx = None
    if need_dx:
        dx = dx_acc if dx_acc is not None else _empty(T * M, I, dev=dev)
    n_part = lib().ptv_gru_persist_part_elems(2, M, H, S) if S else 0
    tens = {'X': xf, 'DOUT': dout, 'DX': dx, 'SYNC': _persist_sync(2, dev)}
    for d_ in range(2):
        dgi, dgh, _, _ = _bigru_bwd_buffers(state, T, M, H, dev)
        tens.update({'HALL%d' % d_: state.hall[d_], 'H16_%d' % d_: state.h16[d_], 'GATES%d' % d_: state.gates[d_], 'WT_HH%d' % d_: wts[d_],
                     'WT_IH%d' % d_: wt_ih[d_], 'DGI%d' % d_: dgi, 'DGH%d' % d_: dgh,
                     'XCH%d' % d_: torch.empty(T * M * 3 * H, device=dev, dtype=BF16),
                     'PART%d' % d_: torch.empty(n_part, device=dev) if S else None})
    evs = _fork_events('BGB')
    turn = _CompositeTurn(cur_stream())
    slots = _BGB.pointers(tens, dict(zip(_BIGRU_G, G)), handles={'FORK_EVENT': evs[0].cuda_event, 'JOIN_EVENT': evs[1].cuda_event,
                                                                 'SIDE_STREAM': side.s.cuda_stream, **turn.handles})
    rc = lib().ptv_bigru_final_bwd(slots, _BGB.dims(dims), stream_ptr())
    _SIDE_DEPTH[1] = 1
    if rc == -3:
        raise RuntimeError('ptv_bigru_final_bwd refused a configuration its Python-side checks accepted')
    check(rc, 'ptv_bigru_final_bwd')
    turn.taken()
    _BGB.count()
    return G[0:4] + G[4:8], (dx.view(T, M, I) if need_dx else None)


def _bigru_backward(prec, x3, w, state, dout, need_dx, dx_acc=None, rev_slot=None):
    T, M, I = x3.shape
    H = w[1].shape[1]
    dev = x3.device
    xf = x3.reshape(T * M, I)
    branch = state.branch
    if branch == 'rows' and not (NOTES_PERSIST and prec == 1 and BF16_STORAGE):
        raise RuntimeError("bi-GRU backward: the forward ran on the row kernels (BiGruState.branch == 'rows') and they cannot run now "
                           '(NOTES_PERSIST / bf16 precision): no other BPTT reads their gate layout')
    wts = [_WT(w[1], prec), _WT(w[5], prec)]
    if branch == 'persist' and not (wts[0] is not None and wts[1] is not None and persist_supported(2, M, H, T)):
        branch = 'step'
    late = {}

    def dx_of(d, dgi2, top, first):
        if not need_dx:
            return None
        if first and dx_acc is None:
# ... 607 lines not shown
        else:
            side.join()
        if res.ev_dtoks is not None:
            if len(_SUMMARY_EV) > 8:
                _SUMMARY_EV.clear()
            _SUMMARY_EV[dTOKS[1:].data_ptr()] = res.ev_dtoks
        demb_out = demb.view(16, 32, B, E)
        if ctx.emb_link is not None and ctx.needs_input_grad[2] and demb.dtype == F32 and demb.is_contiguous():
            ctx.emb_link['demb'] = demb
            demb_out = None
        return (dz, demb_out, dTOKS[1:].view(R, 2 * He), None, None, None) + tuple(G[n] for n in DEC_PARAM_NAMES)


DEC_BWD_COMPOSITE = os.environ.get('PTV_BWD_COMPOSITES', '1') != '0'
_DTB = SlotTable('DTB')
_DTB_G = tuple(('G_' + k, n) for k, n in (
          ('W_ZHID', 'z2dec_hid_linear.weight'), ('B_ZHID', 'z2dec_hid_linear.bias'), ('W_ZIN', 'z2dec_in_linear.weight'),
          ('B_ZIN', 'z2dec_in_linear.bias'), ('INIT_INPUT', 'dec_init_input'), ('W_IH_T', 'dec_time_gru.weight_ih_l0'),
          ('W_HH_T', 'dec_time_gru.weight_hh_l0'), ('B_IH_T', 'dec_time_gru.bias_ih_l0'), ('B_HH_T', 'dec_time_gru.bias_hh_l0'),
          ('W_T2N', 'dec_time_to_notes_hid.weight'), ('B_T2N', 'dec_time_to_notes_hid.bias'), ('W_IH_N', 'dec_notes_gru.weight_ih_l0'),
          ('W_HH_N', 'dec_notes_gru.weight_hh_l0'), ('B_IH_N', 'dec_notes_gru.bias_ih_l0'), ('B_HH_N', 'dec_notes_gru.bias_hh_l0'),
          ('W_P', 'pitch_out_linear.weight'), ('B_P', 'pitch_out_linear.bias'), ('W_DH', 'dur_hid_linear.weight'),
          ('B_DH', 'dur_hid_linear.bias'), ('W_OUT_D', 'dur_out_linear.weight'), ('B_OUT_D', 'dur_out_linear.bias'),
          ('W_IH_D', 'dec_dur_gru.weight_ih_l0'), ('W_HH_D', 'dec_dur_gru.weight_hh_l0'), ('B_IH_D', 'dec_dur_gru.bias_ih_l0'),
          ('B_HH_D', 'dec_dur_gru.bias_hh_l0'), ('SOS', 'dur_sos_token')))


def decoder_bwd_composite_static_ok(prec, B, Ht, Hn, NP, Hd, E, P=None):
    return (prec == 1 and ZERO_SKIP and OVERLAP and SUMMARY_FAMILY_SLOT < 0 and DEC_BWD_COMPOSITE and not torch.cuda.is_current_stream_capturing()
            and DUR_RECOMPUTE and HEADS_WGRAD_FUSED and HEADS_FUSED and BF16_STORAGE and (Hn, NP, Hd) == (512, 130, 64)
            and notes_persist_ok(prec, Hn, E, BF16) and persist_supported(1, B, Ht, 32)
            and 15 * 32 * B * 5 >= 4096
            and (P is None or all(_WT(P[n], prec) is not None for n in (
                'dec_notes_gru.weight_ih_l0', 'dec_time_to_notes_hid.weight', 'dec_time_gru.weight_ih_l0', 'dec_time_gru.weight_hh_l0',
                'z2dec_hid_linear.weight', 'z2dec_in_linear.weight'))))


DecoderGrads = collections.namedtuple('DecoderGrads', 'dz dtok dTOKS G side ev_dtoks')


def _decoder_bwd_composite(P, st, z, tok_op, dP, ddur, top_h, side, G):
    B, R, E, He, Ht, Hn, Hd, NP, prec = st.B, st.R, st.E, st.He, st.Ht, st.Hn, st.Hd, st.NP, st.prec
    dev = z.device
    M = 15 * R
    if (not decoder_bwd_composite_static_ok(prec, B, Ht, Hn, NP, Hd, E, P)
            or (st.notes, st.heads, st.dur) != ('rows', 'fused', 'fused16') or st.gates_d is not None or st.NS16 is None
            or dP.stride(0) != _pad8(NP) or dP.data_ptr() % 16 or not ddur.is_contiguous() or ddur.dtype != F32
            or tok_op.dtype != F32 or not tok_op.is_contiguous() or z.dtype != F32 or not z.is_contiguous() or side.s == side.main):
        _defer_flush()
        return None
    wts = [_WT(P[n], prec) for n in ('dec_notes_gru.weight_ih_l0', 'dec_time_to_notes_hid.weight', 'dec_time_gru.weight_ih_l0',
                                      'dec_time_gru.weight_hh_l0', 'z2dec_hid_linear.weight', 'z2dec_in_linear.weight')]
    HN16, HD16, NS16, gates_n, gates_t = st.HN16, st.HD16, st.NS16, st.gates_n, st.gates_t
    Zs, Zi = z.shape[1], st.z_in.shape[1]
    S = persist_splitk(1, B, Ht)
    nblk = min(256, (M + 63) // 64)
    psz = lib().ptv_dur_gru_bwd_part_size()
    dims = {'B': B, 'E': E, 'HE': He, 'HT': Ht, 'HN': Hn, 'HD': Hd, 'NP': NP, 'ZS': Zs, 'ZI': Zi, 'LDP': _pad8(NP), 'NBLK': nblk, 'SPLITK': S}
    hp = heads_packs(P['pitch_out_linear.weight'], P['dur_hid_linear.weight'])
    pk = notes_packs(P['dec_notes_gru.weight_ih_l0'], P['dec_notes_gru.weight_hh_l0'], Ht)
    for _, n in _DTB_G:
        G[n] = _gbuf(P[n])
    dz, dtok, dTOKS = _empty(B, Zs, dev=dev), _empty(16, R, E, dev=dev), _empty(33, B, 2 * He, dev=dev)
    tab0, tab = st.dur_tabs
    tens = {'Z': z, 'TOK_OP': tok_op, 'DP': dP, 'DDUR': ddur, 'TOP_H': top_h,
            'W_HH_D': P['dec_dur_gru.weight_hh_l0'], 'B_HH_D': P['dec_dur_gru.bias_hh_l0'], 'W_IH_D': P['dec_dur_gru.weight_ih_l0'],
            'W_OUT_D': P['dur_out_linear.weight'], 'SOS': P['dur_sos_token'], 'PK_WDPT': hp['wdpT'], 'PK_WCAT': hp['wcat'],
            'PK_NOTES_WT': pk['wt'], 'WT_IH_N': wts[0], 'WT_T2N': wts[1], 'WT_IH_T': wts[2], 'WT_HH_T': wts[3], 'WT_ZHID': wts[4],
            'WT_ZIN': wts[5], 'NS': st.NS, 'NS16': NS16, 'Z_IN': st.z_in, 'TOKS': st.TOKS, 'GATES_T': gates_t, 'HN16': HN16,
            'GATES_N': gates_n, 'PITCH': st.pitch, 'HD16': HD16, 'TAB0': tab0, 'TAB': tab, 'IDX': st.idx,
            'DZ': dz, 'DTOK': dtok, 'DTOKS': dTOKS,
            'DHD0': _empty(M, Hd, dev=dev), 'PART': _empty(nblk, psz, dev=dev), 'S': _zeros(1, psz, dev=dev), 'TMP64': _zeros(1, 64, dev=dev),
            'DNSUM': _empty(M, Hn, dev=dev, dtype=BF16), 'DY16': _empty(M, 200, dev=dev, dtype=BF16), 'TMP200': _empty(200, Hn, dev=dev),
            'CS200': _zeros(200, dev=dev), 'DGI_N': _empty(15, R, 3 * Hn, dev=dev, dtype=BF16), 'DGH_N': _empty(15, R, Hn, dev=dev, dtype=BF16),
            'DHN0': _empty(R, Hn, dev=dev), 'SCRATCH_N': _empty(lib().ptv_notes_gru_persist_scratch_elems(R), dev=dev, dtype=BF16),
            'TOP_STEP': _ineg1(dev), 'DGC': _empty(R, 3 * Hn, dev=dev), 'DNS': _empty(R, Ht, dev=dev),
            'DGI_T': _empty(32, B, 3 * Ht, dev=dev, dtype=BF16), 'DGH_T': _empty(32, B, 3 * Ht, dev=dev, dtype=BF16),
            'DZHID': _empty(B, Ht, dev=dev), 'DZG': _empty(B, 3 * Ht, dev=dev), 'DZ_IN': _empty(B, Zi, dev=dev),
            'XCH': torch.empty(32 * B * 3 * Ht, device=dev, dtype=BF16),
            'PART_T': torch.empty(lib().ptv_gru_persist_part_elems(1, B, Ht, S), device=dev) if S else None,
            'SYNC': _persist_sync(1, dev)}
    srt = st.sorted
    if srt is not None:
        tens.update(PERM=srt.perm, ROW_LEN=srt.len, NS16S=srt.NS16S, TOK_OP=srt.TOK_S.view(M, E), DNS_S=_empty(R, Ht, dev=dev),
                    DTOK_S=_empty(15, R, E, dev=dev), SEG_N=srt.seg_n)
    if POISON_DEAD_STEPS and top_h is not None and st.live_top is not None:
        _poison(tens['DNSUM'], tens['DGI_N'], tens['DGH_N'], tens['DY16'])
    evs = _fork_events('DTB', 4)
    turn = _CompositeTurn(cur_stream())
    arr_ = _DTB.pointers(tens, {k: G[n] for k, n in _DTB_G},
                         handles={'FORK_EVENT0': evs[0].cuda_event, 'FORK_EVENT1': evs[1].cuda_event, 'FORK_EVENT2': evs[2].cuda_event,
                                  'FORK_EVENT3': evs[3].cuda_event, 'SIDE_STREAM': side.s.cuda_stream, **turn.handles})
    mark('dec_bwd:composite')
    darr_, sp_ = _DTB.dims(dims), stream_ptr()
    rc = _defer_or_run('tf_bwd', (arr_, darr_, tens, turn.prev, turn.done, evs), lambda: lib().ptv_decoder_tf_bwd(arr_, darr_, sp_))
    _SIDE_DEPTH[1] = 1
    if rc == -3:
        raise RuntimeError('ptv_decoder_tf_bwd refused a configuration its Python-side checks accepted')
    check(rc, 'ptv_decoder_tf_bwd')
    turn.taken()
    _DTB.count()
    side.used = True
    side.keep.extend([v for k, v in tens.items() if v is not None] + [st, z, tok_op])
    return DecoderGrads(dz, dtok, dTOKS, G, side, None)


def decoder_bwd_core(P, st, z, tok_op, dpitch, ddur):
    B, R, E, He, Ht, Hn, Hd, NP, prec = st.B, st.R, st.E, st.He, st.Ht, st.Hn, st.Hd, st.NP, st.prec
    if st.notes == 'rows' and not notes_persist_ok(prec, Hn, E):
        raise RuntimeError("decoder backward: the forward ran on the row kernel (DecoderState.notes == 'rows') and it cannot run now "
                           '(NOTES_PERSIST or BF16_STORAGE switched off since): only csrc/notes_persist.hip reads its gate planes')
    dev = z.device
    M = 15 * R
    G = {n: None for n in DEC_PARAM_NAMES}
    NS, HN, HD, TOKS = st.NS, st.HN, st.HD, st.TOKS
    NSo = st.NS16 if st.NS16 is not None else NS
    HNo = st.HN16 if st.HN16 is not None else HN
    HDo = st.HD16 if st.HD16 is not None else HD
    NSf_op, NSUM_op = NSo[1:].view(R, Ht), HNo[1:].view(M, Hn)
    side = Side(DEC_WGRAD_SLOT)

    def wgrad(name, dy, x, sub=None):
        if G[name] is None:
            G[name] = _gbuf(P[name])
        out = G[name] if sub is None else G[name][:, sub]
        gemm(dy, x, out, ta=True, tb=True, acc=True, prec=prec)

    def bgrad(name, a):
        G[name] = _bgrad(P[name], a)

    def wgrad_b(name, bname, dy, x, sub=None, k_top=None):
        if G[name] is None:
            G[name] = _gbuf(P[name])
        if bname is not None and G[bname] is None:
            G[bname] = _gbuf(P[bname])
        wgrad_bias(dy, x, G[name] if sub is None else G[name][:, sub], G[bname] if bname is not None else None, prec, k_top, R)

    hint = _loss_top_hint(dpitch, ddur)
    ddur = (ddur.contiguous() if ddur is not None else _zeros(M, 5, 2, dev=dev)).view(M, 10)
    if (DP_INPLACE and dpitch is not None and dpitch.dtype == F32 and _row_dense(dpitch) and dpitch.stride(-2) == _pad8(NP)
            and dpitch.numel() == M * NP and not dpitch.requires_grad):
        dP = _rows2d(dpitch)
    else:
        dP = _empty(M, _pad8(NP), dev=dev)[:, :NP]
        if dpitch is not None:
            copy2d(dP, _rows2d(dpitch))
        else:
            copy2d(dP, _zeros(1, NP, dev=dev), lds=0)

    mark('dec_bwd:start')
    zero_skip_sync()
    top_h = None
    if ZERO_SKIP:
        if st.live_top is not None:
            top_h = st.live_top
        elif hint is not None:
            top_h = hint
        else:
            top_h = _ineg1(dev)
            call('ptv_last_nonzero_unit', ptr(dP), M, NP, dP.stride(0), R, ptr(top_h), stream_ptr())
            call('ptv_last_nonzero_unit', ptr(ddur), M, 10, 10, R, ptr(top_h), stream_ptr())

    res = _decoder_bwd_composite(P, st, z, tok_op, dP, ddur, top_h, side, G)
    if res is not None:
        return res
    if st.sorted is not None:
        raise RuntimeError('the decoder forward ran on length-sorted rows (PTV_SORT_DEC_ROWS) but ptv_decoder_tf_bwd, the only place that '
                           'restores the row order, declined this backward pass')
# ... 320 lines not shown
    tp = [t.permute(*p) for t, p in zip(ts, perms)]
    if all(t.is_contiguous() or _row_dense(t) for t in tp):
        return tp, True
    return [t.contiguous() for t in ts], False


WDUR = (1.0, 0.6, 0.4, 0.3, 0.3)


def _pianotree_ce_fwd(pitch_m, dur_m, sm, x, sums, st, weighted=False, targets=None):
    dev = pitch_m.device
    B = x.shape[0]
    rows = B * 480
    NP = pitch_m.shape[-1]
    if targets is not None:
        pitch_t, dur_t, counts = targets
    else:
        pitch_t = torch.empty(rows, device=dev, dtype=torch.int32)
        dur_t = torch.empty(rows * 5, device=dev, dtype=torch.int32)
        counts = _izeros(3, dev)
        call('ptv_pianotree_targets', ptr(x), B, int(sm), ptr(pitch_t), ptr(dur_t), ptr(counts), st)
    call('ptv_ce_fwd', ptr(pitch_m), pitch_m.stride(-2), ptr(pitch_t), rows, NP, 130, ptr(sums[0:]), st)
    if weighted:
        gsum = _zeros(5, dev=dev)
        gcnt = _izeros(5, dev)
        call('ptv_ce_group_fwd', ptr(dur_m), 2, ptr(dur_t), rows * 5, 2, 2, 5, ptr(gsum), ptr(gcnt), st)
        call('ptv_wdur_finalize', ptr(gsum), ptr(gcnt), *WDUR, ptr(sums[1:]), ptr(counts[1:]), st)
        return pitch_t, dur_t, counts, gcnt
    call('ptv_ce_fwd', ptr(dur_m), 2, ptr(dur_t), rows * 5, 2, 2, ptr(sums[1:]), st)
    return pitch_t, dur_t, counts, None


def _pianotree_ce_bwd(pitch_m, dur_m, sm, pitch_t, dur_t, gs, st, gcnt=None):
    NP = pitch_m.shape[-1]
    rows = pitch_t.numel()
    ld = pitch_m.stride(-2)
    dpitch = torch.empty(rows, ld, device=pitch_m.device)[:, :NP].as_strided(pitch_m.shape, pitch_m.stride())
    ddur = torch.empty_like(dur_m)
    call('ptv_ce_bwd', ptr(pitch_m), ld, ptr(pitch_t), rows, NP, 130, ptr(gs[0:]), ptr(dpitch), ld, st)
    if gcnt is not None:
        gs5 = _empty(5, dev=pitch_m.device)
        call('ptv_wdur_scales', ptr(gs[1:]), ptr(gcnt), *WDUR, ptr(gs5), st)
        call('ptv_ce_group_bwd', ptr(dur_m), 2, ptr(dur_t), rows * 5, 2, 2, 5, ptr(gs5), ptr(ddur), 2, st)
    else:
        call('ptv_ce_bwd', ptr(dur_m), 2, ptr(dur_t), rows * 5, 2, 2, ptr(gs[1:]), ptr(ddur), 2, st)
    if sm:
        dpitch, ddur = dpitch.permute(*_PERM[4]), ddur.permute(*_PERM[5])
    return dpitch, ddur


_LOSS_TOP = {}

DEAD_STEPS = os.environ.get('PTV_DEAD_STEPS', '1') != '0'
POISON_DEAD_STEPS = False
_LIVE = {}


class LiveRows:

    def __init__(self, x, pitch_t, dur_t, counts, sort=None):
        self.x, self.version = x, x._version
        self.pitch_t, self.dur_t, self.counts = pitch_t, dur_t, counts
        self.top = counts[2:3]
        self.sort = sort
        self.sorted = None

    def record_order(self, sorted):
        if self.sorted is not None or (sorted and self.sort is None):
            raise RuntimeError('LiveRows: row order recorded twice, or sorted without a sort (one plan serves one forward)')
        self.sorted = bool(sorted)

    def targets(self, x, step_major):
        if self.sorted is None:
            raise RuntimeError('LiveRows: no decoder recorded its row order')
        if x.data_ptr() != self.x.data_ptr() or x.shape != self.x.shape or x._version != self.version:
            raise RuntimeError('LiveRows: the loss is given another x than the plan was built for')
        if not step_major:
            raise RuntimeError('LiveRows: the logits are not step-major')
        if self.sorted:
            return self.sort['pt'], self.sort['dt'], self.counts
        return self.pitch_t, self.dur_t, self.counts


def live_rows(x):
    if not (DEAD_STEPS and ZERO_SKIP and x.is_cuda and x.dtype == torch.int64 and x.is_contiguous() and x.shape[0] % 4 == 0):
        return None
    B = x.shape[0]
    R = 32 * B
    sort = SORT_DEC_ROWS and DEC_COMPOSITE and DEC_BWD_COMPOSITE and not torch.cuda.is_current_stream_capturing()
    row_live = _izeros(R, x.device) if sort else None
    pitch_t = torch.empty(B * 480, device=x.device, dtype=torch.int32)
    dur_t = torch.empty(B * 2400, device=x.device, dtype=torch.int32)
    counts = _izeros(3, x.device)
    call('ptv_pianotree_targets_rows', ptr(x), B, 1, ptr(pitch_t), ptr(dur_t), ptr(counts), ptr(row_live), stream_ptr())
    srt = None
    if sort:
        perm = torch.empty(R, device=x.device, dtype=torch.int32)
        call('ptv_rows_by_length', ptr(row_live), ptr(perm), R, 15, stream_ptr())
        len_s = torch.empty(R, device=x.device, dtype=torch.int32)
        call('ptv_gather_rows', ptr(len_s), ptr(row_live), ptr(perm), R, 1, 0, 0, 1, stream_ptr())
        pt_s, dt_s = torch.empty_like(pitch_t), torch.empty_like(dur_t)
        call('ptv_gather_rows', ptr(pt_s), ptr(pitch_t), ptr(perm), R, 1, R, R, 15, stream_ptr())
        call('ptv_gather_rows', ptr(dt_s), ptr(dur_t), ptr(perm), R, 5, 5 * R, 5 * R, 15, stream_ptr())
        seg_n = None
        if WGRAD_SEG and R % 128 == 0 and lib().ptv_wgrad_seg_supported(15 * R, R):
            seg_n = torch.empty(15, device=x.device, dtype=torch.int32)
            call('ptv_rows_seg_counts', ptr(len_s), R, 15, ptr(seg_n), stream_ptr())
            global _LAST_SEG_N
            _LAST_SEG_N = seg_n
        srt = dict(perm=perm, len=len_s, pt=pt_s, dt=dt_s, seg_n=seg_n)
    _LIVE['last_counts'] = counts
    return LiveRows(x, pitch_t, dur_t, counts, srt)


def _poison(*tensors):
    for t in tensors:
        if t is None:
            continue
        if t.dtype.is_floating_point:
            t.fill_(float('nan'))
        else:
            t.fill_(0x3fffffff)


def _loss_top_hint(dpitch, ddur):
    ent = _LOSS_TOP.pop('hint', None)
    if ent is None or dpitch is None or ddur is None:
        return None
    gp, gd, vp, vd, top = ent

    def same(a, b, v):
        return (a.data_ptr() == b.data_ptr() and a.shape == b.shape and a.stride() == b.stride() and a.dtype == b.dtype
                and b._version == v and a._version == v)
    return top if (same(gp, dpitch, vp) and same(gd, ddur, vd)) else None


LOSS_TOP_HINT = True


LOSS_COMPOSITE = os.environ.get('PTV_BWD_COMPOSITES', '1') != '0'
_VL = SlotTable('VL')


def _vl_ok(*ts):
    return all(t.is_cuda and t.dtype == F32 and t.is_contiguous() for t in ts)


def _vae_loss_fwd_composite(pitch_m, dur_m, sm_p, x, c, mu_c, sd_c, mu_r, sd_r, root_m, chroma_m, bass_m, sm_c, root_t, chroma_t, bass_t,
                            targets, sums, out, scal, st):
    B = x.shape[0]
    NP = pitch_m.shape[-1]
    if (x.dtype != torch.int64 or not _vl_ok(c, mu_c, sd_c, mu_r, sd_r, root_m, chroma_m, bass_m) or pitch_m.dtype != F32 or dur_m.dtype != F32
            or not dur_m.is_contiguous() or not _row_dense(pitch_m) or pitch_m.numel() != B * 480 * NP or dur_m.numel() != B * 4800):
        return None
    dev = pitch_m.device
    if targets is not None:
        pitch_t, dur_t, counts = targets
    else:
        pitch_t = torch.empty(B * 480, device=dev, dtype=torch.int32)
        dur_t = torch.empty(B * 2400, device=dev, dtype=torch.int32)
        counts = _izeros(3, dev)
    dims = _VL.dims({'B': B, 'Z': mu_c.shape[1], 'NP': NP, 'LDP': pitch_m.stride(-2), 'SM_P': sm_p, 'SM_C': sm_c,
                     'HAVE_TARGETS': targets is not None})
    slots = _VL.pointers({'X': x, 'C': c, 'PITCH': pitch_m, 'DUR': dur_m, 'MU_C': mu_c, 'SD_C': sd_c, 'MU_R': mu_r, 'SD_R': sd_r,
                          'ROOT': root_m, 'CHROMA': chroma_m, 'BASS': bass_m, 'PITCH_T': pitch_t, 'DUR_T': dur_t, 'COUNTS': counts,
                          'ROOT_T': root_t, 'CHROMA_T': chroma_t, 'BASS_T': bass_t, 'SUMS': sums, 'OUT': out})
    rc = lib().ptv_vae_loss_fwd(slots, dims, (ctypes.c_double * 6)(*scal), st)
    check(rc, 'ptv_vae_loss_fwd')
    _VL.count()
    return pitch_t, dur_t, counts


def _vae_loss_bwd_composite(gout, gs, pitch_m, dur_m, mu_c, sd_c, mu_r, sd_r, root_m, chroma_m, bass_m, pitch_t, dur_t, counts, root_t, chroma_t,
                            bass_t, dpitch, ddur, dmu_c, dsd_c, dmu_r, dsd_r, droot, dchroma, dbass, scal, st):
    B = root_t.numel() // 8
    NP = pitch_m.shape[-1]
    if gout.dtype != F32 or not _row_dense(pitch_m) or not dur_m.is_contiguous():
        return False
    dims = _VL.dims({'B': B, 'Z': mu_c.shape[1], 'NP': NP, 'LDP': pitch_m.stride(-2)})
    slots = _VL.pointers({'PITCH': pitch_m, 'DUR': dur_m, 'MU_C': mu_c, 'SD_C': sd_c, 'MU_R': mu_r, 'SD_R': sd_r, 'ROOT': root_m,
                          'CHROMA': chroma_m, 'BASS': bass_m, 'PITCH_T': pitch_t, 'DUR_T': dur_t, 'COUNTS': counts, 'ROOT_T': root_t,
                          'CHROMA_T': chroma_t, 'BASS_T': bass_t, 'GOUT': gout, 'GS': gs, 'DPITCH': dpitch, 'DDUR': ddur, 'DMU_C': dmu_c,
                          'DSD_C': dsd_c, 'DMU_R': dmu_r, 'DSD_R': dsd_r, 'DROOT': droot, 'DCHROMA': dchroma, 'DBASS': dbass})
    rc = lib().ptv_vae_loss_bwd(slots, dims, (ctypes.c_double * 6)(*scal), st)
    check(rc, 'ptv_vae_loss_bwd')
    _VL.count('bwd_calls')
    return True


class VaeLossFn(torch.autograd.Function):
# ... 208 lines not shown
```

Measured before the change: 82020 samples/s.

## Fuse row-unsort scatter into GEMM epilogue and build row sort plan in one kernel

The decoder backward GEMMs now take a row map and write their outputs straight to the original row order from the epilogue. This removes the separate sorted staging buffers and the two scatter kernels that followed. A new multi-block rows_plan kernel computes the length-sorted permutation, the sorted lengths and the segment counts in one launch, replacing a single-block sort plus gather plus count kernels. The cost is scattered row writes inside the GEMM epilogue, one lane shuffle per row, and a new sort kernel that recounts the histogram in every block.

```diff
diff --git a/include/ptvae_hip.h b/include/ptvae_hip.h
--- a/include/ptvae_hip.h
+++ b/include/ptvae_hip.h
@@ -33,6 +33,10 @@
 int ptv_gemm_mtop_seg(int prec, int transA, int transB, int M, int N, int K, const void* A, long lda, const void* B, long ldb,
                       void* C, long ldc, const float* bias, float alpha, int accumulate, int act, int splitk, int dtypes,
                       const int* m_top, long m_unit, const int* seg_n, long seg_unit, int seg_period, void* stream);
+int ptv_gemm_mtop_seg_map(int prec, int transA, int transB, int M, int N, int K, const void* A, long lda, const void* B, long ldb,
+                          void* C, long ldc, const float* bias, float alpha, int accumulate, int act, int splitk, int dtypes,
+                          const int* m_top, long m_unit, const int* seg_n, long seg_unit, int seg_period,
+                          const int* c_rows, long c_unit, void* stream);
 int ptv_gemm_priority(int p);
 
 int ptv_gru_seq_fwd(int prec, int M, int H, int T,
@@ -318,8 +322,6 @@
   PTV_DTB_FORK_EVENT0, PTV_DTB_FORK_EVENT1, PTV_DTB_FORK_EVENT2, PTV_DTB_FORK_EVENT3,
   PTV_DTB_PERM, PTV_DTB_ROW_LEN,
   PTV_DTB_NS16S,
-  PTV_DTB_DNS_S,
-  PTV_DTB_DTOK_S,
   PTV_DTB_SEG_N,
   PTV_DTB_COUNT
 };
@@ -516,6 +518,8 @@
                                  const float* dh_last, long last_ld, const int* lengths, const int* perm, void* dgi, void* dgh,
                                  float* dh0, void* scratch, long R, int T, int reverse, int* top_step, void* stream);
 int ptv_rows_by_length(const int* lengths, int* perm, long R, int max_len, void* stream);
+#define PTV_ROWS_PLAN_MAX_R 65536
+int ptv_rows_plan(const int* lengths, long R, int max_len, int steps, int* perm, int* len_sorted, int* seg_n, void* stream);
 
 int ptv_cast_bf16(const float* src, void* dst, long n, void* stream);
 int ptv_transpose_cast_bf16(const float* src, void* dst, int rows, int cols, void* stream);
diff --git a/polyphonic_chord_texture_disentanglement_amd/csrc/composite.hip b/polyphonic_chord_texture_disentanglement_amd/csrc/composite.hip
--- a/polyphonic_chord_texture_disentanglement_amd/csrc/composite.hip
+++ b/polyphonic_chord_texture_disentanglement_amd/csrc/composite.hip
@@ -234,11 +234,10 @@
   if (!t || !d) return PTV_ERR_ARG;
   for (int i = 0; i < PTV_DTB_COUNT; i++)
     if (!t[i] && i != PTV_DTB_TOP_H && i != PTV_DTB_PART_T && i != PTV_DTB_WAIT_EVENT && i != PTV_DTB_RECORD_EVENT && i != PTV_DTB_PERM &&
-        i != PTV_DTB_ROW_LEN && i != PTV_DTB_NS16S && i != PTV_DTB_DNS_S && i != PTV_DTB_DTOK_S && i != PTV_DTB_SEG_N)
+        i != PTV_DTB_ROW_LEN && i != PTV_DTB_NS16S && i != PTV_DTB_SEG_N)
       return PTV_ERR_ARG;
   const bool sorted = t[PTV_DTB_PERM] != nullptr;
-  if (sorted != (t[PTV_DTB_ROW_LEN] != nullptr) || sorted != (t[PTV_DTB_NS16S] != nullptr) || sorted != (t[PTV_DTB_DNS_S] != nullptr) ||
-      sorted != (t[PTV_DTB_DTOK_S] != nullptr) || (sorted && !t[PTV_DTB_TOP_H]))
+  if (sorted != (t[PTV_DTB_ROW_LEN] != nullptr) || sorted != (t[PTV_DTB_NS16S] != nullptr) || (sorted && !t[PTV_DTB_TOP_H]))
     return PTV_ERR_ARG;
   const int* perm = (const int*)T_(t, PTV_DTB_PERM);
   const int* row_len = (const int*)T_(t, PTV_DTB_ROW_LEN);
@@ -305,23 +304,19 @@
   void* dgi_n = M_<void>(t, PTV_DTB_DGI_N); void* dgh_n = M_<void>(t, PTV_DTB_DGH_N);
   float* dHN0 = GB(PTV_DTB_DHN0); int* top_step = M_<int>(t, PTV_DTB_TOP_STEP);
   float* dGC = GB(PTV_DTB_DGC);
-  float* dNS_out = GB(PTV_DTB_DNS); float* dtok_out = GB(PTV_DTB_DTOK);
-  float* dNS = sorted ? GB(PTV_DTB_DNS_S) : dNS_out;
-  float* dtok = sorted ? GB(PTV_DTB_DTOK_S) : dtok_out;
+  float* dNS = GB(PTV_DTB_DNS); float* dtok = GB(PTV_DTB_DTOK);
   const __bf16* wt_ih_n = (const __bf16*)T_(t, PTV_DTB_WT_IH_N);
   ptv_gemm_priority(1);
   PTV_TRY(ptv_notes_gru_persist_bwd_rows(T_(t, PTV_DTB_PK_NOTES_WT), T_(t, PTV_DTB_HN16), T_(t, PTV_DTB_GATES_N), dNSUM, dgi_n, dgh_n, dHN0,
                                          M_<void>(t, PTV_DTB_SCRATCH_N), R, 15 | (seg_n ? 0x10000 : 0), top_h, row_len, top_step, stream));
   PTV_TRY(ptv_sum_steps_seg(dGC, dgi_n, (long)R * 3 * Hn, 15, (long)R * 3 * Hn, 0, 1, top_step, seg_n, 3L * Hn, stream));
-  if (hipMemsetAsync(dtok_out + 15L * R * E, 0, sizeof(float) * R * E, s) != hipSuccess) return PTV_ERR_LAUNCH;
-  PTV_TRY(ptv_gemm_mtop_seg(P, 0, 0, (int)M, E, 3 * Hn, dgi_n, 3L * Hn, wt_ih_n + (long)Ht * 3 * Hn, 3L * Hn, dtok, E, nullptr, 1.f, 0, 0, 0, A16 | B16,
-                            top_step, R, seg_n, R, 15, stream));
-  PTV_TRY(ptv_gemm(P, 0, 0, R, Ht, 3 * Hn, dGC, 3L * Hn, wt_ih_n, 3L * Hn, dNS, Ht, nullptr, 1.f, 0, 0, 0, B16, stream));
-  PTV_TRY(ptv_gemm(P, 0, 0, R, Ht, Hn, dHN0, Hn, T_(t, PTV_DTB_WT_T2N), Hn, dNS, Ht, nullptr, 1.f, 1, 0, 0, B16, stream));
-  if (sorted) {
-    PTV_TRY(ptv_scatter_rows(dNS_out, dNS, perm, R, Ht, 0, 0, 1, stream));
-    PTV_TRY(ptv_scatter_rows_seg(dtok_out, dtok, perm, R, E, (long)R * E, (long)R * E, 15, seg_n, stream));
-  }
+  if (hipMemsetAsync(dtok + 15L * R * E, 0, sizeof(float) * R * E, s) != hipSuccess) return PTV_ERR_LAUNCH;
+  PTV_TRY(ptv_gemm_mtop_seg_map(P, 0, 0, (int)M, E, 3 * Hn, dgi_n, 3L * Hn, wt_ih_n + (long)Ht * 3 * Hn, 3L * Hn, dtok, E, nullptr, 1.f, 0, 0, 0, A16 | B16,
+                                top_step, R, seg_n, R, 15, perm, R, stream));
+  PTV_TRY(ptv_gemm_mtop_seg_map(P, 0, 0, R, Ht, 3 * Hn, dGC, 3L * Hn, wt_ih_n, 3L * Hn, dNS, Ht, nullptr, 1.f, 0, 0, 0, B16, nullptr, 0, nullptr, 0, 0,
+                                perm, R, stream));
+  PTV_TRY(ptv_gemm_mtop_seg_map(P, 0, 0, R, Ht, Hn, dHN0, Hn, T_(t, PTV_DTB_WT_T2N), Hn, dNS, Ht, nullptr, 1.f, 1, 0, 0, B16, nullptr, 0, nullptr, 0, 0,
+                                perm, R, stream));
   PTV_TRY(fork(2));
   ptv_gemm_priority(0);
   {
@@ -345,7 +340,7 @@
   {
     const float* hall_[1] = {(const float*)T_(t, PTV_DTB_NS)}; const void* gates_[1] = {T_(t, PTV_DTB_GATES_T)};
     const void* wt_[1] = {T_(t, PTV_DTB_WT_HH_T)};
-    const void* ext_[1] = {dNS_out}; const long ext_step[1] = {(long)B * Ht}, ext_ld[1] = {(long)Ht}; const int ext_bf[1] = {0};
+    const void* ext_[1] = {dNS}; const long ext_step[1] = {(long)B * Ht}, ext_ld[1] = {(long)Ht}; const int ext_bf[1] = {0};
     const float* last_[1] = {nullptr}; const long last_ld[1] = {0};
     void* dgi_[1] = {dgi_t}; void* dgh_[1] = {dgh_t}; float* dh0_[1] = {dzhid}; const int rev[1] = {0};
     void* xch_[1] = {M_<void>(t, PTV_DTB_XCH)}; float* part_[1] = {M_<float>(t, PTV_DTB_PART_T)};
diff --git a/polyphonic_chord_texture_disentanglement_amd/csrc/gemm.hip b/polyphonic_chord_texture_disentanglement_amd/csrc/gemm.hip
--- a/polyphonic_chord_texture_disentanglement_amd/csrc/gemm.hip
+++ b/polyphonic_chord_texture_disentanglement_amd/csrc/gemm.hip
@@ -7,30 +7,47 @@
 
 namespace ptv {
 
-struct EpiPlain {
-  struct Params {
-    void* C; long ldc;
-    const float* bias;
-    float alpha;
-    int accumulate;
-    int act;
-    int atomic;
-    int c_bf16;
-    int c_blocked;
-    int c_rows;
-    long split_stride;
-  };
+struct EpiPlainParams {
+  void* C; long ldc;
+  const float* bias;
+  float alpha;
+  int accumulate;
+  int act;
+  int atomic;
+  int c_bf16;
+  int c_blocked;
+  int c_brows;
+  long split_stride;
+  const int* c_rows; int c_unit;
+};
+template <bool MAP>
+struct EpiPlainT {
+  using Params = EpiPlainParams;
   static __device__ __forceinline__ long coff(const Params& p, int m, int n) {
-    return p.c_blocked ? (((long)(n >> p.c_blocked) * p.c_rows + m) << p.c_blocked) + (n & ((1 << p.c_blocked) - 1)) : (long)m * p.ldc + n;
+    return p.c_blocked ? (((long)(n >> p.c_blocked) * p.c_brows + m) << p.c_blocked) + (n & ((1 << p.c_blocked) - 1)) : (long)m * p.ldc + n;
   }
   static __device__ __forceinline__ bool dead_is_noop(const Params& p) { return (p.accumulate || p.atomic) && p.act == 0 && p.bias == nullptr; }
-  template <int FM, int FN, int NG> struct Pre {};
+  template <bool, int DUMMY = 0> struct PreRows {};
+  template <int DUMMY> struct PreRows<true, DUMMY> { int r; };
+  template <int FM, int FN, int NG> struct Pre : PreRows<MAP> {};
   template <int FM, int FN, int NG>
-  static __device__ __forceinline__ void prefetch(const Params&, Pre<FM, FN, NG>&, int, int, int, int) {}
+  static __device__ __forceinline__ void prefetch(const Params& p, Pre<FM, FN, NG>& pre, int m0, int, int M, int) {
+    if constexpr (MAP) {
+      static_assert(16 * FM <= 64, "one lane per row of the wave tile");
+      const int lane = threadIdx.x & 63, m = m0 + lane;
+      pre.r = m;
+      if (lane < 16 * FM && m < M) { const int base = (m / p.c_unit) * p.c_unit; pre.r = base + p.c_rows[m - base]; }
+    }
+  }
+  template <int FM, int FN, int NG>
+  static __device__ __forceinline__ int crow(const Pre<FM, FN, NG>& pre, int m0, int r) {
+    if constexpr (MAP) return __shfl(pre.r, r, 64);
+    else return m0 + r;
+  }
   template <int FN> static constexpr bool staged() { return FN == 2 || FN == 4; }
   template <int FM, int FN, int NG> static constexpr int lds_bytes() { return staged<FN>() ? 4 * RowStage<1, (staged<FN>() ? FN * 16 : 64)>::WAVE_BYTES : 0; }
   template <int FM, int FN, int NG>
-  static __device__ __forceinline__ void apply(const Params& p_in, f32x4 (&acc)[FM][NG * FN], const Pre<FM, FN, NG>&,
+  static __device__ __forceinline__ void apply(const Params& p_in, f32x4 (&acc)[FM][NG * FN], const Pre<FM, FN, NG>& pre,
                                                int m0, int n0, int M, int N, int split, char* lds) {
     Params q = p_in;
     if (q.split_stride) q.C = reinterpret_cast<float*>(q.C) + (long)split * q.split_stride;
@@ -47,11 +64,11 @@
         const int mode = p.atomic ? 3 : (p.accumulate ? (bf ? 4 : 2) : (bf ? 1 : 0));
         float4 b4 = make_float4(0.f, 0.f, 0.f, 0.f);
         if (use_bias) b4 = *reinterpret_cast<const float4*>(p.bias + n0 + u);
-        if (mode == 0) fast_rows<FM, FN, 0>(p, acc, st, m0, n0 + u, b4);
-        else if (mode == 1) fast_rows<FM, FN, 1>(p, acc, st, m0, n0 + u, b4);
-        else if (mode == 2) fast_rows<FM, FN, 2>(p, acc, st, m0, n0 + u, b4);
-        else if (mode == 4) fast_rows<FM, FN, 4>(p, acc, st, m0, n0 + u, b4);
-        else fast_rows<FM, FN, 3>(p, acc, st, m0, n0 + u, b4);
+        if (mode == 0) fast_rows<FM, FN, 0>(p, acc, pre, st, m0, n0 + u, b4);
+        else if (mode == 1) fast_rows<FM, FN, 1>(p, acc, pre, st, m0, n0 + u, b4);
+        else if (mode == 2) fast_rows<FM, FN, 2>(p, acc, pre, st, m0, n0 + u, b4);
+        else if (mode == 4) fast_rows<FM, FN, 4>(p, acc, pre, st, m0, n0 + u, b4);
+        else fast_rows<FM, FN, 3>(p, acc, pre, st, m0, n0 + u, b4);
         return;
       }
 #pragma unroll
@@ -60,7 +77,8 @@
 #pragma unroll
         for (int c = 0; c < RS::PASSES; c++) {
           const int row = RS::row(c), m = m0 + i * 16 + row, n = n0 + u;
-          if (m < M && n < N) cell(p, m, n, N, RS::get(st, row, u), bf, vec, use_bias);
+          const int mc = crow(pre, m0, i * 16 + row);
+          if (m < M && n < N) cell(p, mc, n, N, RS::get(st, row, u), bf, vec, use_bias);
         }
         __builtin_amdgcn_wave_barrier();
       }
@@ -71,12 +89,14 @@
 #pragma unroll
         for (int j = 0; j < FN; j++) {
           const int m = m0 + i * 16 + (lane & 15), n = n0 + j * 16 + (lane >> 4) * 4;
-          if (m < M && n < N) cell(p, m, n, N, acc[i][j], bf, vec, use_bias);
+          const int mc = crow(pre, m0, i * 16 + (lane & 15));
+          if (m < M && n < N) cell(p, mc, n, N, acc[i][j], bf, vec, use_bias);
         }
     }
   }
   template <int FM, int FN, int MODE>
-  static __device__ __forceinline__ void fast_rows(const Params& p, f32x4 (&acc)[FM][FN], float* st, int m0, int n, const float4& b4) {
+  static __device__ __forceinline__ void fast_rows(const Params& p, f32x4 (&acc)[FM][FN], const Pre<FM, FN, 1>& pre, float* st, int m0, int n,
+                                                   const float4& b4) {
     using RS = RowStage<1, FN * 16>;
     const int u = RS::unit();
 #pragma unroll
@@ -86,7 +106,7 @@
       for (int c = 0; c < RS::PASSES; c++) {
         const int row = RS::row(c);
         const f32x4 a = RS::get(st, row, u);
-        const long off = coff(p, m0 + i * 16 + row, n);
+        const long off = coff(p, crow(pre, m0, i * 16 + row), n);
         float v0 = p.alpha * a[0] + b4.x, v1 = p.alpha * a[1] + b4.y, v2 = p.alpha * a[2] + b4.z, v3 = p.alpha * a[3] + b4.w;
         if constexpr (MODE == 1 || MODE == 4) {
           if constexpr (MODE == 4) {
@@ -130,6 +150,8 @@
   }
 };
 
+using EpiPlain = EpiPlainT<false>;
+
 #ifndef PTV_PF_TN
 #define PTV_PF_TN 3
 #endif
@@ -144,12 +166,21 @@
   gemm_body<CT, BM, BN, WGM, WGN, 1, KA, KB, EpiPlain, SA, SB, (BM * BN <= 64 * 64 ? 2 : PLAIN_PF_BIG(KA, KB, SA, SB))>(g, ep);
 }
 
-__global__ void splitk_reduce_kernel(float* __restrict__ C, long ldc, const float* __restrict__ ws, int M, int N, int splits, int accumulate) {
+template <class CT, int BM, int BN, int WGM, int WGN, bool KB, bool SA, bool SB>
+__global__ __launch_bounds__(NTHREADS, 2) void gemm_plain_map_kernel(GemmArgs g, EpiPlainParams ep) {
+  if (g.prio) __builtin_amdgcn_s_setprio(3);
+  gemm_body<CT, BM, BN, WGM, WGN, 1, false, KB, EpiPlainT<true>, SA, SB, (BM * BN <= 64 * 64 ? 2 : PLAIN_PF_BIG(false, KB, SA, SB))>(g, ep);
+}
+
+__global__ void splitk_reduce_kernel(float* __restrict__ C, long ldc, const float* __restrict__ ws, int M, int N, int splits, int accumulate,
+                                     const int* __restrict__ c_rows, int c_unit) {
   const long total = (long)M * N;
   for (long i = (long)blockIdx.x * blockDim.x + threadIdx.x; i < total; i += (long)gridDim.x * blockDim.x) {
     float sum = 0.f;
     for (int z = 0; z < splits; z++) sum += ws[(long)z * total + i];
-    float* cp = C + (i / N) * ldc + (i % N);
+    long m = i / N;
+    if (c_rows) { const long base = (m / c_unit) * c_unit; m = base + c_rows[m - base]; }
+    float* cp = C + m * ldc + (i % N);
     *cp = (accumulate ? *cp : 0.f) + sum;
   }
 }
@@ -163,6 +194,12 @@
 template <class CT, int BM, int BN, bool KA, bool KB, bool SA, bool SB>
 static void launch_plain(const GemmArgs& g, const EpiPlain::Params& ep, int splits, hipStream_t s) {
   dim3 grid(cdiv(g.N, BN), cdiv(g.M, BM), splits);
+  if constexpr (!KA) {
+    if (ep.c_rows) {
+      hipLaunchKernelGGL((gemm_plain_map_kernel<CT, BM, BN, 2, 2, KB, SA, SB>), grid, dim3(NTHREADS), 0, s, g, ep);
+      return;
+    }
+  }
   hipLaunchKernelGGL((gemm_plain_kernel<CT, BM, BN, 2, 2, KA, KB, SA, SB>), grid, dim3(NTHREADS), 0, s, g, ep);
 }
 
@@ -224,6 +261,7 @@
   }
   if (ws) {
     ep.C = ws; ep.ldc = g.N; ep.accumulate = 0; ep.atomic = 0; ep.split_stride = (long)g.M * g.N;
+    ep.c_rows = nullptr; ep.c_unit = 0;
   } else if (splits > 1) {
     ep.atomic = 1;
     if (!ep.accumulate) {
@@ -245,7 +283,8 @@
   if (ws) {
     const long total = (long)g.M * g.N;
     int nb = (int)((total + 255) / 256); if (nb > 2048) nb = 2048;
-    hipLaunchKernelGGL(splitk_reduce_kernel, dim3(nb), dim3(256), 0, s, reinterpret_cast<float*>(ep_user.C), ep_user.ldc, ws, g.M, g.N, splits, ep_user.accumulate);
+    hipLaunchKernelGGL(splitk_reduce_kernel, dim3(nb), dim3(256), 0, s, reinterpret_cast<float*>(ep_user.C), ep_user.ldc, ws, g.M, g.N, splits, ep_user.accumulate,
+                       ep_user.c_rows, ep_user.c_unit);
   }
   return PTV_OK;
 }
@@ -268,7 +307,17 @@
                                  void* C, long ldc, const float* bias, float alpha,
                                  int accumulate, int act, int splitk, int dtypes, const int* m_top, long m_unit,
                                  const int* seg_n, long seg_unit, int seg_period, void* stream) {
+  return ptv_gemm_mtop_seg_map(prec, transA, transB, M, N, K, A, lda, B, ldb, C, ldc, bias, alpha, accumulate, act, splitk, dtypes, m_top, m_unit, seg_n,
+                               seg_unit, seg_period, nullptr, 0, stream);
+}
+
+extern "C" int ptv_gemm_mtop_seg_map(int prec, int transA, int transB, int M, int N, int K,
+                                     const void* A, long lda, const void* B, long ldb,
+                                     void* C, long ldc, const float* bias, float alpha,
+                                     int accumulate, int act, int splitk, int dtypes, const int* m_top, long m_unit,
+                                     const int* seg_n, long seg_unit, int seg_period, const int* c_rows, long c_unit, void* stream) {
   if (M < 0 || N < 0 || K < 0 || !A || !B || !C) return PTV_ERR_ARG;
+  if (c_rows && ((dtypes & 24) || splitk > 1 || transA || c_unit <= 0 || c_unit > 0x7fffffffL || M % c_unit != 0)) return PTV_ERR_ARG;
   if (M == 0 || N == 0) return PTV_OK;
   const bool sa = dtypes & 1, sb = dtypes & 2, sc = dtypes & 4;
   if ((sa || sb) && prec != PTV_PREC_BF16) return PTV_ERR_ARG;
@@ -283,7 +332,7 @@
   if (m_top && (transA || m_unit <= 0)) return PTV_ERR_ARG;
   if (seg_n && (transA || seg_unit <= 0 || (seg_unit & 127) || seg_period <= 0)) return PTV_ERR_ARG;
   ptv::GemmArgs g{A, lda, B, ldb, M, N, K, K, 0, m_top, m_unit, ptv::g_gemm_prio, seg_n, (int)seg_unit, seg_period};
-  ptv::EpiPlain::Params ep{C, ldc, bias, alpha, accumulate, act, 0, sc ? 1 : 0, (dtypes & 8) ? 5 : ((dtypes & 16) ? 4 : 0), M, 0};
+  ptv::EpiPlain::Params ep{C, ldc, bias, alpha, accumulate, act, 0, sc ? 1 : 0, (dtypes & 8) ? 5 : ((dtypes & 16) ? 4 : 0), M, 0, c_rows, c_rows ? (int)c_unit : 0};
   hipStream_t s = (hipStream_t)stream;
   int rc;
   if (prec != PTV_PREC_BF16) rc = ptv::gemm_dispatch<ptv::F32, false, false>(transA, transB, g, ep, splitk, s);
diff --git a/polyphonic_chord_texture_disentanglement_amd/csrc/notes_persist.hip b/polyphonic_chord_texture_disentanglement_amd/csrc/notes_persist.hip
--- a/polyphonic_chord_texture_disentanglement_amd/csrc/notes_persist.hip
+++ b/polyphonic_chord_texture_disentanglement_amd/csrc/notes_persist.hip
@@ -622,6 +622,66 @@
   }
 }
 
+constexpr int PLAN_ROWS = 256, PLAN_MAX_BINS = 39;
+__global__ __launch_bounds__(PLAN_ROWS) void rows_plan_kernel(const int* __restrict__ lengths, int R, int nb, int steps, int* __restrict__ perm,
+                                                              int* __restrict__ len_sorted, int* __restrict__ seg_n) {
+  __shared__ int cnt[PLAN_MAX_BINS * PLAN_ROWS];
+  __shared__ int before[PLAN_MAX_BINS], total[PLAN_MAX_BINS], wcnt[4][PLAN_MAX_BINS + 1];
+  const int tid = threadIdx.x, lane = tid & 63, wave = tid >> 6;
+  const int nchunk = (R + PLAN_ROWS - 1) / PLAN_ROWS, mine = blockIdx.x;
+  for (int b = 0; b < nb; b++) cnt[b * PLAN_ROWS + tid] = 0;
+  auto bin_of = [&](int r) { return r < R ? min(max(lengths[r], 0), nb - 1) : -1; };
+  auto count = [&](int c0, int c1) {
+    for (int c = c0; c < c1; c += 16) {
+      int q[16];
+#pragma unroll
+      for (int j = 0; j < 16; j++) {
+        const int r = (c + j) * PLAN_ROWS + tid;
+        const bool ok = c + j < c1 && r < R;
+        const int v = lengths[ok ? r : 0];
+        q[j] = ok ? min(max(v, 0), nb - 1) : -1;
+      }
+#pragma unroll
+      for (int j = 0; j < 16; j++)
+        if (q[j] >= 0) atomicAdd(&cnt[q[j] * PLAN_ROWS + tid], 1);
+    }
+  };
+  auto reduce = [&](int* out) {
+    __syncthreads();
+    for (int b = wave; b < nb; b += 4) {
+      int v = cnt[b * PLAN_ROWS + lane] + cnt[b * PLAN_ROWS + 64 + lane] + cnt[b * PLAN_ROWS + 128 + lane] + cnt[b * PLAN_ROWS + 192 + lane];
+#pragma unroll
+      for (int d = 32; d >= 1; d >>= 1) v += __shfl_xor(v, d, 64);
+      if (lane == 0) out[b] = v;
+    }
+    __syncthreads();
+  };
+  count(0, mine);
+  reduce(before);
+  count(mine, nchunk);
+  reduce(total);
+  const int r = mine * PLAN_ROWS + tid, q = bin_of(r);
+  int rank = 0;
+  for (int b = 0; b < nb; b++) {
+    const unsigned long long m = __ballot(q == b);
+    if (q == b) rank = __popcll(m & ((1ull << lane) - 1ull));
+    if (lane == 0) wcnt[wave][b] = __popcll(m);
+  }
+  __syncthreads();
+  if (q >= 0) {
+    int pos = before[q] + rank;
+    for (int b = q + 1; b < nb; b++) pos += total[b];
+    for (int w = 0; w < wave; w++) pos += wcnt[w][q];
+    perm[pos] = r;
+    if (len_sorted) len_sorted[pos] = q;
+  }
+  if (seg_n && mine == 0 && tid < steps) {
+    int live = 0;
+    for (int b = tid + 1; b < nb; b++) live += total[b];
+    seg_n[tid] = (live + 127) / 128 * 128;
+  }
+}
+
 }
 
 using namespace ptv;
@@ -637,6 +697,17 @@
     attr = true;
   }
   hipLaunchKernelGGL(rows_by_length_kernel, dim3(1), dim3(1024), lds, (hipStream_t)stream, lengths, perm, R, nb);
+  PTV_CHECK_LAUNCH();
+  return PTV_OK;
+}
+
+extern "C" int ptv_rows_plan(const int* lengths, long R, int max_len, int steps, int* perm, int* len_sorted, int* seg_n, void* stream) {
+  if (!lengths || !perm || R <= 0 || R > 0x7fffffffL || max_len < 0) return PTV_ERR_ARG;
+  if (seg_n && ((R & 127) || steps <= 0 || steps > 64)) return PTV_ERR_ARG;
+  if (max_len + 1 > PLAN_MAX_BINS) return PTV_ERR_UNSUPPORTED;
+  if (R > PTV_ROWS_PLAN_MAX_R) return PTV_ERR_UNSUPPORTED;
+  hipLaunchKernelGGL(rows_plan_kernel, dim3((unsigned)((R + PLAN_ROWS - 1) / PLAN_ROWS)), dim3(PLAN_ROWS), 0, (hipStream_t)stream, lengths, (int)R,
+                     max_len + 1, seg_n ? steps : 0, perm, len_sorted, seg_n);
   PTV_CHECK_LAUNCH();
   return PTV_OK;
 }
diff --git a/polyphonic_chord_texture_disentanglement_amd/functional.py b/polyphonic_chord_texture_disentanglement_amd/functional.py
--- a/polyphonic_chord_texture_disentanglement_amd/functional.py
+++ b/polyphonic_chord_texture_disentanglement_amd/functional.py
@@ -1055,13 +1055,8 @@
     if branch == 'rows':
         skip_by = lengths if ZERO_SKIP else None
         if lengths is not None and ZERO_SKIP and SORT_ROWS and T <= 38:
-            perm = torch.empty(M, device=dev, dtype=torch.int32)
-            call('ptv_rows_by_length', ptr(lengths), ptr(perm), M, T, stream_ptr())
-            if WGRAD_SEG and M % 128 == 0 and lib().ptv_wgrad_seg_supported(T * M, M):
-                len_s = torch.empty(M, device=dev, dtype=torch.int32)
-                call('ptv_gather_rows', ptr(len_s), ptr(lengths), ptr(perm), M, 1, 0, 0, 1, stream_ptr())
-                seg = torch.empty(T, device=dev, dtype=torch.int32)
-                call('ptv_rows_seg_counts', ptr(len_s), M, T, ptr(seg), stream_ptr())
+            want_seg = bool(WGRAD_SEG and M % 128 == 0 and lib().ptv_wgrad_seg_supported(T * M, M))
+            perm, _, seg = rows_plan(lengths, M, T, T, want_seg, want_len=False)
         if BIGRU_BWD_COMPOSITE:
             state = _bigru_rows_fwd_composite(x3, lengths, skip_by, perm, seg, w, out, side, T, M, I, H, dev)
             if state is not None:
@@ -1835,8 +1830,7 @@
             'SYNC': _persist_sync(1, dev)}
     srt = st.sorted
     if srt is not None:
-        tens.update(PERM=srt.perm, ROW_LEN=srt.len, NS16S=srt.NS16S, TOK_OP=srt.TOK_S.view(M, E), DNS_S=_empty(R, Ht, dev=dev),
-                    DTOK_S=_empty(15, R, E, dev=dev), SEG_N=srt.seg_n)
+        tens.update(PERM=srt.perm, ROW_LEN=srt.len, NS16S=srt.NS16S, TOK_OP=srt.TOK_S.view(M, E), SEG_N=srt.seg_n)
     if POISON_DEAD_STEPS and top_h is not None and st.live_top is not None:
         _poison(tens['DNSUM'], tens['DGI_N'], tens['DGH_N'], tens['DY16'])
     evs = _fork_events('DTB', 4)
@@ -2323,6 +2317,26 @@
         return self.pitch_t, self.dur_t, self.counts
 
 
+ROWS_PLAN_MAX_R = 65536
+
+
+def rows_plan(lengths, R, max_len, steps, want_seg, want_len=True):
+    dev = lengths.device
+    perm = torch.empty(R, device=dev, dtype=torch.int32)
+    plan = R <= ROWS_PLAN_MAX_R
+    len_s = torch.empty(R, device=dev, dtype=torch.int32) if (want_len or (want_seg and not plan)) else None
+    seg = torch.empty(steps, device=dev, dtype=torch.int32) if want_seg else None
+    if plan:
+        call('ptv_rows_plan', ptr(lengths), R, max_len, steps, ptr(perm), ptr(len_s), ptr(seg), stream_ptr())
+    else:
+        call('ptv_rows_by_length', ptr(lengths), ptr(perm), R, max_len, stream_ptr())
+        if len_s is not None:
+            call('ptv_gather_rows', ptr(len_s), ptr(lengths), ptr(perm), R, 1, 0, 0, 1, stream_ptr())
+        if seg is not None:
+            call('ptv_rows_seg_counts', ptr(len_s), R, steps, ptr(seg), stream_ptr())
+    return perm, len_s, seg
+
+
 def live_rows(x):
     if not (DEAD_STEPS and ZERO_SKIP and x.is_cuda and x.dtype == torch.int64 and x.is_contiguous() and x.shape[0] % 4 == 0):
         return None
@@ -2336,17 +2350,12 @@
     call('ptv_pianotree_targets_rows', ptr(x), B, 1, ptr(pitch_t), ptr(dur_t), ptr(counts), ptr(row_live), stream_ptr())
     srt = None
     if sort:
-        perm = torch.empty(R, device=x.device, dtype=torch.int32)
-        call('ptv_rows_by_length', ptr(row_live), ptr(perm), R, 15, stream_ptr())
-        len_s = torch.empty(R, device=x.device, dtype=torch.int32)
-        call('ptv_gather_rows', ptr(len_s), ptr(row_live), ptr(perm), R, 1, 0, 0, 1, stream_ptr())
+        want_seg = bool(WGRAD_SEG and R % 128 == 0 and lib().ptv_wgrad_seg_supported(15 * R, R))
+        perm, len_s, seg_n = rows_plan(row_live, R, 15, 15, want_seg)
         pt_s, dt_s = torch.empty_like(pitch_t), torch.empty_like(dur_t)
         call('ptv_gather_rows', ptr(pt_s), ptr(pitch_t), ptr(perm), R, 1, R, R, 15, stream_ptr())
         call('ptv_gather_rows', ptr(dt_s), ptr(dur_t), ptr(perm), R, 5, 5 * R, 5 * R, 15, stream_ptr())
-        seg_n = None
-        if WGRAD_SEG and R % 128 == 0 and lib().ptv_wgrad_seg_supported(15 * R, R):
-            seg_n = torch.empty(15, device=x.device, dtype=torch.int32)
-            call('ptv_rows_seg_counts', ptr(len_s), R, 15, ptr(seg_n), stream_ptr())
+        if seg_n is not None:
             global _LAST_SEG_N
             _LAST_SEG_N = seg_n
         srt = dict(perm=perm, len=len_s, pt=pt_s, dt=dt_s, seg_n=seg_n)
```

Result: faster. 83340 samples/s (median of 6 runs) (+1.6%).
